# kris927b/TextBlaster

Measured on AMD Instinct MI355X. Metric: documents/sec through full C4+Gopher+langID pipeline at 1/2/4/8 MI355X, higher is better.
Workload: dtype bf16

## Files before the change

csrc/common/devplan.h:

```cpp
#pragma once
#include "tb_common.h"

namespace tb {

constexpr int kMaxStageSteps = 8;
constexpr int kMaxNgramEntries = 16;
constexpr int kMaxStopChars = 16;
constexpr int kMaxStopWords = 512;
constexpr int kStopTableSize = 2048;
constexpr int kStopBlobBytes = 16384;

enum DevStepKind : int32_t {
  DK_NONE = 0,
  DK_GOPHER_QUALITY = 1,
  DK_GOPHER_REP = 2,
  DK_FINEWEB = 3,
  DK_LANGID = 4,
};

constexpr uint32_t kC4MaxGrowth = 16;

struct DevStep {
  int32_t kind;
  int32_t width;
  int64_t rec_base;
  int32_t rec_prefix;
  int32_t stop_set;
  int32_t n_top, n_dup;
  int32_t top_n[kMaxNgramEntries];
  int32_t dup_n[kMaxNgramEntries];
  int32_t n_stop_chars;
  uint32_t stop_chars[kMaxStopChars];
  int64_t short_line_length;
};

constexpr int kStopLiteMaxSlots = 256;
constexpr int kStopLiteMaxWords = 64;
constexpr int kStopLiteMaxBlob = 1024;

TB_HD uint32_t stop_lite_hash_push(uint32_t h, uint8_t v) { return (h ^ v) * 16777619u; }
constexpr uint32_t kStopLiteHash0 = 2166136261u;
TB_HD uint32_t stop_lite_slot(uint32_t h, uint32_t nslots) { return (h * 0x9E3779B1u) & (nslots - 1); }

struct DevStopSet {
  uint64_t keys[kStopTableSize];
  int32_t idx[kStopTableSize];
  int32_t off[kMaxStopWords + 1];
  int32_t n;
  int32_t max_len;
  uint8_t blob[kStopBlobBytes];
  int32_t lite_nslots;
  uint32_t lite_slots[kStopLiteMaxSlots];
  uint64_t fast_keys[kStopLiteMaxSlots];
  int32_t all_ascii7;
};

TB_HD uint32_t stop_fast_slot(uint64_t key, uint32_t nslots) {
  uint64_t h = key * 0x9E3779B97F4A7C15ull;
  return (uint32_t)(h >> 40) & (nslots - 1);
}

struct DevC4 {
  int32_t split_paragraph, remove_citations, filter_no_terminal_punct;
  int32_t filter_lorem_ipsum, filter_javascript, filter_curly_bracket, filter_policy;
  int64_t min_words_per_line, max_word_length;
  int64_t min_num_sentences;
};

struct DevStage {
  int32_t n_steps;
  int32_t width_total;
  DevStep steps[kMaxStageSteps];
};

constexpr int kMaxStopSets = 4;

struct DevPlan {
  int32_t n_stop_sets;
  DevStopSet stops[kMaxStopSets];
};

constexpr uint64_t kScratchPerByte = 80;
constexpr uint64_t kScratchPerByteSplit = 176;
TB_HD uint64_t scratch_bytes_for_dev(uint32_t doc_len, bool split = false) {
  return (split ? kScratchPerByteSplit : kScratchPerByte) * ((uint64_t)doc_len + 64) + 4096;
}

TB_HD uint64_t dev_key(uint64_t h, uint32_t len) {
  uint64_t x = h ^ ((uint64_t)len * 0xD6E8FEB86659FD93ull);
  x ^= x >> 33;
  x *= 0xff51afd7ed558ccdull;
  x ^= x >> 33;
  x *= 0xc4ceb9fe1a85ec53ull;
  x ^= x >> 33;
  return x | 1ull;
}

constexpr uint32_t kNoWords = 0xFFFFFFFFu;
struct DictLines {
  const int64_t* off = nullptr;
  const uint32_t* data = nullptr;
  TB_HD const uint32_t* at(uint32_t d) const { return (off && off[d] >= 0) ? data + off[d] : nullptr; }
};
struct DictIn {
  const int64_t* moff = nullptr;
  const uint32_t* bits = nullptr;
  const uint32_t* words = nullptr;
  TB_HD const uint32_t* marks(uint32_t d) const { return (moff && moff[d] >= 0) ? bits + moff[d] : nullptr; }
  TB_HD uint32_t nwords(uint32_t d) const { return words ? words[d] : kNoWords; }
};

}
```

csrc/common/docproc.h:

```cpp
#pragma once
#include <type_traits>

#include "devplan.h"
#include "hash.h"
#include "langid.h"
#include "par.h"
#include "uax29.h"
#include "ucd.h"

namespace tb {

enum : int {
  PH_START = 0, PH_DECODE, PH_DICT, PH_PREFIX_HASH, PH_WORDS, PH_LINES, PH_GQ, PH_GR_LINES, PH_GR_WORDS,
  PH_GR_TOP, PH_GR_DUP, PH_FW, PH_LID, PH_GR_DUP_WALK, PH_GR_DUP_CANON, PH_GR_TOP_CANON,
  PH_C4_LOREM = 16, PH_C4_DECODE, PH_C4_LINES, PH_C4_CITE, PH_C4_WORDS, PH_C4_CODES, PH_C4_JOIN, PH_C4_SENT,
  PH_GR_NL = 24, PH_GR_LINE_DUP, PH_GR_WH, PH_GR_WCANON, PH_GQ_WORDS, PH_GQ_BYTES, PH_RUST_LINES,
  kPhaseSlots = 32
};

enum : uint32_t {
  DOC_OK = 0,
  DOC_NEEDS_CPU = 1,
  DOC_OVERFLOW = 2,
};

constexpr uint32_t P16_CASE_IGN = 1u << 14;
TB_HD uint16_t compact_prop(uint32_t p) {
  return (uint16_t)((p & 0xBFFFu) | ((p & P_CASE_IGN) ? P16_CASE_IGN : 0u));
}

struct PropArr {
  const uint32_t* ent = nullptr;
  const uint16_t* p16 = nullptr;
  TB_HD uint32_t operator[](uint32_t i) const { return ent ? (ent[i] >> 16) : (uint32_t)p16[i]; }
  TB_HD PropArr operator+(uint32_t s) const { return PropArr{ent ? ent + s : nullptr, ent ? nullptr : p16 + s}; }
};
struct OffArr {
  const uint32_t* ent = nullptr;
  const uint32_t* o32 = nullptr;
  TB_HD uint32_t operator[](uint32_t i) const { return ent ? (ent[i] & 0xFFFFu) : o32[i]; }
};

struct Cps {
  uint32_t n = 0;
  uint32_t* ent = nullptr;
  uint32_t* off = nullptr;
  uint16_t* prop = nullptr;
  const uint8_t* b = nullptr;
  uint32_t nb = 0;
  TB_HD PropArr props() const { return PropArr{ent, prop}; }
  TB_HD OffArr offs() const { return OffArr{ent, off}; }
  TB_HD uint32_t o(uint32_t i) const { return ent ? (ent[i] & 0xFFFFu) : off[i]; }
  TB_HD uint32_t p(uint32_t i) const { return ent ? (ent[i] >> 16) : (uint32_t)prop[i]; }
  TB_HD uint8_t lead(uint32_t i) const { return b[o(i)]; }
  TB_HD bool is_lf(uint32_t i) const { return (p(i) & P_WB_MASK) == (uint32_t)WB_LF; }
  TB_HD uint32_t cp(uint32_t i) const {
    int len;
    return utf8_decode(b, o(i), nb, &len);
  }
};

struct CpsAcc {
  PropArr prop;
  TB_HD uint32_t p(int i) const { return prop[(uint32_t)i]; }
};

struct PHView {
  const uint64_t* ph8 = nullptr;
  uint64_t phn = 0;
  const uint8_t* b = nullptr;
  uint32_t n = 0;
  TB_HD uint64_t at(uint32_t x) const {
    if (x >= n) return phn;
    uint64_t h = ph8[x >> 3];
    for (uint32_t j = x & ~7u; j < x; ++j) h = hash_push(h, b[j]);
    return h;
  }
};

struct PreDoc {
  uint32_t* off;
  uint16_t* prop;
  uint32_t* wbm;
  uint32_t* nl_pos;
  uint32_t* nl_len;
  uint32_t n;
  uint32_t C;
  uint32_t dict;
  uint32_t NL;
  uint32_t tcs;
  uint32_t tce;
  uint32_t nl_a;
  uint32_t nl_e;
  uint32_t* wtmp;
  uint32_t* wcs;
  uint32_t* wce;
  uint32_t* wbs;
  uint32_t* wbe;
  uint8_t* wal;
  uint32_t W;
  uint32_t pad;
  uint64_t* wh;
  uint64_t* wtab;
  uint64_t* wk;
  uint64_t* wpb;
  uint64_t* wcsum;
  uint32_t* wslot;
  uint32_t* wid;
  uint32_t* wl;
  uint32_t wready;
  uint32_t pad2;
};

struct Words {
  uint32_t n = 0;
  uint32_t* cs = nullptr;
  uint32_t* ce = nullptr;
  uint32_t* bs = nullptr;
  uint32_t* be = nullptr;
  uint8_t* alpha = nullptr;
};

struct Lines {
  uint32_t n = 0;
  uint32_t* ls = nullptr;
  uint32_t* le = nullptr;
};

struct HL {
  uint64_t h;
  uint32_t len;
  uint32_t pad;
};

template <class P>
struct DocCtx {
  P par;
  UcdView ucd;
  const uint64_t* pw = nullptr;
  const uint64_t* ipw = nullptr;
  uint32_t pw_n = 0;
// ... 68 lines not shown
    uint64_t a = (used + 15) & ~15ull;
    uint64_t e = a + count * sizeof(T) + 16;
    if (e > cap) {
      overflow = true;
      return (T*)scr;
    }
    used = a + count * sizeof(T);
    if constexpr (P::kWaves == 0) {
      if (used > peak) peak = used;
    }
    return (T*)(scr + a);
  }
  TB_HD void set_flag(uint32_t f) {
    if (flag) P::or32(flag, f);
  }
  TB_HD uint64_t powb(uint32_t k) const { return k <= pw_n ? pw[k] : hpow(kHashBase, k); }
  TB_HD uint64_t ipowb(uint32_t k) const { return (ipw && k <= pw_n) ? ipw[k] : hpow(kHashBaseInv, k); }
  template <class T>
  TB_HD T* try_lds(uint64_t count) {
    if (!lds) return nullptr;
    const uint64_t a = (lused + 15u) & ~15u;
    const uint64_t e = a + count * sizeof(T);
    if (e + lhi > lcap) return nullptr;
    lused = (uint32_t)e;
    return (T*)(lds + a);
  }
};

TB_HD bool is_ws(uint32_t p) { return (p & P_WS) != 0; }

template <class P, class PA>
TB_HD void trim_span(DocCtx<P>& x, const PA& prop, uint32_t C, uint32_t& tcs, uint32_t& tce) {
#if defined(__HIPCC__)
  if constexpr (P::kWaves == 1) {
    const uint32_t lane = x.par.lane;
    tcs = C;
    for (uint32_t base = 0; base < C; base += 64) {
      const uint32_t j = base + lane;
      const uint64_t m = __ballot(j < C && !is_ws(prop[j]));
      if (m) { tcs = base + (uint32_t)__builtin_ctzll(m); break; }
    }
    tce = 0;
    if (tcs < C) {
      for (uint32_t base = (C - 1) & ~63u;; base -= 64) {
        const uint32_t j = base + lane;
        const uint64_t m = __ballot(j < C && !is_ws(prop[j]));
        if (m) { tce = base + (uint32_t)(64 - __clzll((long long)m)); break; }
        if (base == 0) break;
      }
    }
    return;
  }
#endif
  tcs = x.par.template min<uint32_t>(C, C, [&](uint32_t i) { return is_ws(prop[i]) ? C : i; });
  tce = x.par.template max<uint32_t>(C, 0u, [&](uint32_t i) { return is_ws(prop[i]) ? 0u : i + 1; });
}
constexpr uint32_t kWave16 = 43000;
TB_HD constexpr int rec_gr_fixed() { return 7; }

template <class P>
TB_HD Cps decode(DocCtx<P>& x, const uint8_t* b, uint32_t n, bool hot = false, uint32_t* dict = nullptr) {
  Cps c;
  c.b = b;
  c.nb = n;
  const bool packed = n < 65536u;
  if (packed) {
    c.ent = hot ? x.template alloc_hot_hi<uint32_t>(n + 1) : x.template alloc<uint32_t>(n + 1);
  } else {
    c.prop = hot ? x.template alloc_hot_hi<uint16_t>(n + 1) : x.template alloc<uint16_t>(n + 1);
    c.off = hot ? x.template alloc_hot_hi<uint32_t>(n + 1) : x.template alloc<uint32_t>(n + 1);
  }
  if (x.overflow) return c;
  const UcdView ucd = x.ucd;
  const uint16_t* asc = x.asc;
  uint32_t* ent = c.ent;
  uint32_t* off = c.off;
  uint16_t* pra = c.prop;
  uint32_t dl = 0;
  c.n = x.par.template compact<int>(
      n, [&](uint32_t i, int&) { return utf8_is_lead(b[i]); },
      [&](uint32_t i, uint32_t k, int&) {
        uint16_t cpk;
        const uint32_t c0 = b[i];
        if (asc && (c0 < 0x80 || (c0 & 0xFEu) == 0xC2u)) {
          cpk = asc[c0 < 0x80 ? c0 : (((c0 & 0x1Fu) << 6) | (b[i + 1] & 0x3Fu))];
        } else {
          int len;
          const uint32_t p = ucd.props(utf8_decode(b, i, n, &len));
          cpk = compact_prop(p);
          dl |= (p & P_DICT) ? 1u : 0u;
        }
        if (packed) {
          ent[k] = i | ((uint32_t)cpk << 16);
        } else {
          off[k] = i;
          pra[k] = cpk;
        }
      });
  const uint32_t cn = c.n;
  x.par.single([&]() {
    if (packed) ent[cn] = n;
    else { off[cn] = n; pra[cn] = 0; }
  });
  if (dict) *dict = x.par.reduce_or(dl);
  x.par.sync();
  return c;
}

template <class P>
TB_HD uint64_t span_hash8(const DocCtx<P>& x, const PHView& v, uint32_t s, uint32_t e) {
  const uint64_t hs = v.at(s), he = v.at(e);
  return he - hs * x.powb(e - s);
}

template <class P>
TB_HD PHView prefix_hash8(DocCtx<P>& x, const uint8_t* b, uint32_t n) {
  PHView v;
  v.b = b;
  v.n = n;
  const uint32_t nblk = (n + 7) >> 3;
  uint64_t* ph8 = x.template alloc_hot_hi<uint64_t>(nblk + 1);
  if (x.overflow) return v;
  const uint64_t* pw = x.pw;
  const uint32_t pwn = x.pw_n;
  HL tot = x.par.template scan<HL>(
      nblk, HL{0, 0, 0},
      [&](const HL& a, const HL& c) {
        uint64_t m = c.len <= pwn ? pw[c.len] : hpow(kHashBase, c.len);
        return HL{a.h * m + c.h, a.len + c.len, 0};
      },
      [&](uint32_t k) {
        const uint32_t s0 = k << 3, e0 = s0 + 8 < n ? s0 + 8 : n;
        uint64_t h = 0;
        for (uint32_t j = s0; j < e0; ++j) h = hash_push(h, b[j]);
        return HL{h, e0 - s0, 0};
      },
      [&](uint32_t k, const HL& e) { ph8[k] = e.h; });
  x.par.single([&]() { ph8[nblk] = tot.h; });
  x.par.sync();
  v.ph8 = ph8;
  v.phn = tot.h;
  return v;
}

struct WSeg {
  uint32_t bits;
  uint32_t first;
  uint32_t last;
};
TB_HD WSeg wseg_op(const WSeg& a, const WSeg& b) {
  if (b.bits & 1u) return b;
  return WSeg{a.bits | (b.bits & 6u), a.first < b.first ? a.first : b.first, a.last > b.last ? a.last : b.last};
}

#ifndef TB_WB_CTX
#define TB_WB_CTX 1
#endif
#if defined(__HIPCC__)
static __constant__ WbPairTab g_wb_pair_tab = kWbPairTab;
#endif
TB_HD bool word_mark(const PropArr& prop, uint32_t C, uint32_t i) {
  if (i == 0 || i == C) return true;
  if (TB_WB_CTX) {
    const uint32_t pm2 = i >= 2 ? prop[i - 2] : 0xFFFFFFFFu;
    const uint32_t pp1 = i + 1 < C ? prop[i + 1] : 0xFFFFFFFFu;
#if defined(__HIP_DEVICE_COMPILE__)
    const int r = wb_break_ctx_tab(pm2, prop[i - 1], prop[i], pp1, [](uint32_t k) { return g_wb_pair_tab.w[k]; });
// ... 362 lines not shown
    while (true) {
      uint64_t cur = tab[slot];
      if (cur == 0) {
        cur = P::cas64(&tab[slot], 0, mine);
        if (cur == 0) break;
      }
      if ((cur >> 32) == fp) {
        if ((cur & 0xFFFFFFFFull) > (uint64_t)i + 1u) P::min64(&tab[slot], mine);
        break;
      }
      if (++slot == capn) slot = 0;
    }
    canon[i] = slot;
  });
  x.par.sync();
  bool collided = false;
  x.par.for_n(n, [&](uint32_t i) {
    uint32_t c = (uint32_t)(tab[canon[i]] & 0xFFFFFFFFull) - 1u;
    if (c != i && !eq(i, c)) { collided = true; c = i; }
    canon[i] = c;
    res(i, c);
  });
  if (collided) x.set_flag(DOC_NEEDS_CPU);
  x.par.sync();
  x.reset(mark);
}

template <class P, class KeyF, class EqF, class CT>
TB_HD void canonicalize(DocCtx<P>& x, uint32_t n, KeyF&& key, EqF&& eq, CT* canon) {
  canonicalize_res(x, n, key, eq, canon, NoResolve{});
}

template <class P>
TB_HD bool bytes_eq(const uint8_t* b, uint32_t a0, uint32_t a1, uint32_t b0, uint32_t b1) {
  if (a1 - a0 != b1 - b0) return false;
  const uint32_t n = a1 - a0;
  uint32_t i = 0;
  for (; i + 16 <= n; i += 16) {
    uint32_t diff = 0;
#pragma unroll
    for (uint32_t k = 0; k < 16; ++k) diff |= (uint32_t)(b[a0 + i + k] ^ b[b0 + i + k]);
    if (diff) return false;
  }
  uint32_t diff = 0;
  for (; i < n; ++i) diff |= (uint32_t)(b[a0 + i] ^ b[b0 + i]);
  return diff == 0;
}

template <class P, class SpanF>
TB_HD void dup_spans(DocCtx<P>& x, const uint8_t* b, const PHView& ph, uint32_t n, SpanF&& span,
                     int64_t* out_elems, int64_t* out_bytes) {
  if (n <= 1) {
    *out_elems = 0;
    *out_bytes = 0;
    return;
  }
  const auto mark = x.mark();
  uint32_t* canon = x.template alloc_hot<uint32_t>(n + 1);
  if (x.overflow) return;
  canonicalize(
      x, n,
      [&](uint32_t i) {
        uint32_t s, e;
        span(i, s, e);
        return dev_key(span_hash8(x, ph, s, e), e - s);
      },
      [&](uint32_t i, uint32_t j) {
        uint32_t s0, e0, s1, e1;
        span(i, s0, e0);
        span(j, s1, e1);
        return bytes_eq<P>(b, s0, e0, s1, e1);
      },
      canon);
  *out_elems = x.par.template sum<int64_t>(n, [&](uint32_t i) { return canon[i] != i ? (int64_t)1 : (int64_t)0; });
  *out_bytes = x.par.template sum<int64_t>(n, [&](uint32_t i) {
    if (canon[i] == i) return (int64_t)0;
    uint32_t s, e;
    span(i, s, e);
    return (int64_t)(e - s);
  });
  x.reset(mark);
}

template <class F>
TB_HD void lower_bytes(const UcdView& ucd, const Cps& cv, uint32_t s, uint32_t e, F&& push) {
  uint8_t buf[4];
  const PropArr prop = cv.props();
  for (uint32_t k = s; k < e; ++k) {
    uint32_t c = cv.cp(k);
    uint32_t lc;
    if (c == 0x3A3) {
      bool before = false, after = false;
      for (uint32_t j = k; j > s; --j) {
        uint32_t p = prop[j - 1];
        if (p & P16_CASE_IGN) continue;
        before = (p & P_CASED) != 0;
        break;
      }
      for (uint32_t j = k + 1; j < e; ++j) {
        uint32_t p = prop[j];
        if (p & P16_CASE_IGN) continue;
        after = (p & P_CASED) != 0;
        break;
      }
      lc = (before && !after) ? 0x3C2 : 0x3C3;
    } else {
      lc = ucd.lower(c);
    }
    int nb = utf8_encode(lc, buf);
    for (int q = 0; q < nb; ++q) push(buf[q]);
    if (c == 0x130) { push(0xCC); push(0x87); }
  }
}

TB_HD bool is_stop_word(const UcdView& ucd, const DevStopSet& ss, const Cps& cv, uint32_t s, uint32_t e,
                        uint32_t b0, uint32_t b1) {
  if (ss.n == 0 || (int32_t)(e - s) > ss.max_len) return false;
  if (ss.lite_nslots > 0) {
    const uint32_t nb = b1 - b0;
    if (nb <= 7u && nb == e - s) {
      uint64_t key = (uint64_t)nb << 56;
      for (uint32_t k = 0; k < nb; ++k) {
        uint32_t c = cv.b[b0 + k];
        if (c >= 'A' && c <= 'Z') c += 32;
        key |= (uint64_t)c << (8 * k);
      }
      const uint32_t ns = (uint32_t)ss.lite_nslots;
      uint32_t slot = stop_fast_slot(key, ns);
      while (true) {
        const uint64_t f = ss.fast_keys[slot];
        if (f == 0) return false;
        if (f == key) return true;
        slot = (slot + 1) & (ns - 1);
      }
    }
    if (ss.all_ascii7) {
      bool e2 = false;
      for (uint32_t k = b0; k < b1; ++k) e2 |= cv.b[k] == 0xE2;
      if (!e2) return false;
    }
  }
  uint64_t h = 0;
  uint32_t len = 0;
  lower_bytes(ucd, cv, s, e, [&](uint8_t v) { h = hash_push(h, v); ++len; });
  const uint64_t key = dev_key(h, len);
  uint32_t slot = (uint32_t)(key >> 17) & (kStopTableSize - 1);
  while (true) {
    const uint64_t k = ss.keys[slot];
    if (k == 0) return false;
    if (k == key) {
      const int32_t w = ss.idx[slot];
      const int32_t o0 = ss.off[w], o1 = ss.off[w + 1];
      if ((uint32_t)(o1 - o0) != len) return false;
      int32_t pos = o0;
      bool ok = true;
      lower_bytes(ucd, cv, s, e, [&](uint8_t v) { ok = ok && ss.blob[pos++] == v; });
      return ok;
    }
    slot = (slot + 1) & (kStopTableSize - 1);
  }
}

TB_HD bool ci_contains(const uint8_t* b, uint32_t n, const char* pat, int plen) {
  for (uint32_t s = 0; s < n; ++s) {
    uint32_t i = s;
    int j = 0;
    for (; j < plen; ++j) {
      if (i >= n) break;
      const char pc = pat[j];
      uint8_t c = b[i];
      if (c >= 'A' && c <= 'Z') c = (uint8_t)(c + 32);
      if (c == (uint8_t)pc) { ++i; continue; }
      if (pc == 'k' && i + 2 < n && b[i] == 0xE2 && b[i + 1] == 0x84 && b[i + 2] == 0xAA) { i += 3; continue; }
      break;
    }
    if (j == plen) return true;
  }
  return false;
}

struct GrExport {
  const uint32_t* wid;
  const uint32_t* WL;
  const uint64_t* K;
  const uint64_t* PB;
  const uint32_t* bs;
  const uint32_t* be;
  const uint8_t* b;
  char* free_base;
  uint64_t free_cap;
  uint32_t W;
  uint32_t valid;
  const uint32_t* rs;
  const uint32_t* rl;
  const uint32_t* prs;
  OffArr off;
  PHView ph;
  uint32_t NR, NPR, tcs, tce;
  uint32_t lines_valid;
};

TB_HD void gr_line_span(const uint32_t* rs, const uint32_t* rl, const OffArr& off, uint32_t tcs, uint32_t tce,
                        uint32_t NR, uint32_t k, uint32_t& s0, uint32_t& e0) {
  const uint32_t cs = k == 0 ? tcs : rs[k - 1] + rl[k - 1];
  const uint32_t ce = k == NR ? tce : rs[k];
  s0 = off[cs];
  e0 = off[ce];
}
TB_HD void gr_para_span(const uint32_t* rs, const uint32_t* rl, const uint32_t* prs, const OffArr& off,
                        uint32_t tcs, uint32_t tce, uint32_t NPR, uint32_t q, uint32_t& s0, uint32_t& e0) {
  const uint32_t cs = q == 0 ? tcs : rs[prs[q - 1]] + rl[prs[q - 1]];
  const uint32_t ce = q == NPR ? tce : rs[prs[q]];
  s0 = off[cs];
  e0 = off[ce];
}

struct StageOut {
  int64_t* rec;
  uint32_t ndocs;
  uint32_t doc;
  GrExport* gr_export = nullptr;
  uint32_t* line_stats = nullptr;
  const PreDoc* pre = nullptr;
  const uint8_t* b_global = nullptr;
  DictIn dict;
};

constexpr uint32_t kLineStatsNone = 0xFFFFFFFFu;
struct alignas(16) LineStat { uint32_t bs, be, nw, mx; };
TB_HD uint64_t line_stats_base(int64_t off_d, int64_t d) { return 4ull * ((uint64_t)off_d / 8u + 16ull * (uint64_t)d); }
TB_HD uint32_t line_stats_cap(uint32_t n) { return n / 8u + 15u; }
TB_HD uint64_t line_stats_words(const int64_t* off, int64_t ndocs) {
  return line_stats_base(off[ndocs], ndocs) + 16u;
}

template <class P>
TB_HD void export_line_stats(DocCtx<P>& x, const Cps& c, const Words& w, const Lines& L, uint32_t n, uint32_t* out) {
  const uint32_t NL = L.n;
  if (NL > line_stats_cap(n) || x.overflow) return;
  const auto mark = x.mark();
  uint32_t* ls = x.template alloc_hot<uint32_t>(NL + 1);
  uint32_t* nw = x.template alloc_hot<uint32_t>(NL + 1);
  uint32_t* mx = x.template alloc_hot<uint32_t>(NL + 1);
  if (x.overflow) {
    x.overflow = false;
    x.reset(mark);
    return;
  }
  const PropArr prop = c.props();
  const OffArr off = c.offs();
  x.par.for_n(NL, [&](uint32_t k) { ls[k] = L.ls[k]; nw[k] = 0; mx[k] = 0; });
  x.par.sync();
  x.par.for_n(w.n, [&](uint32_t q) {
    const uint32_t cs = w.cs[q];
    uint32_t lo = 0, hi = NL;
    while (hi - lo > 1) {
      const uint32_t mid = (lo + hi) >> 1;
      if (ls[mid] <= cs) lo = mid; else hi = mid;
    }
    P::add32(&nw[lo], 1u);
    P::max32(&mx[lo], w.ce[q] - cs);
  });
  x.par.sync();
  LineStat* st = (LineStat*)(out + 4);
  x.par.for_n(NL, [&](uint32_t k) {
    uint32_t s0 = ls[k], e0 = L.le[k];
    while (s0 < e0 && is_ws(prop[s0])) ++s0;
    while (e0 > s0 && is_ws(prop[e0 - 1])) --e0;
    st[k] = LineStat{off[s0], off[e0], nw[k], mx[k]};
  });
  x.par.sync();
  x.par.single([&]() { out[0] = NL; });
  x.reset(mark);
}

struct DupGrams {
  const uint32_t* wid;
  const uint32_t* WL;
  const uint64_t* K;
  const uint64_t* PB;
  const uint32_t* bs;
  const uint32_t* be;
// ... 80 lines not shown
      g = gc[p];
      len = WL[p + n] - WL[p];
    }
    const bool seen0 =
        act && ((__hip_atomic_load(&sn[g >> 5], __ATOMIC_RELAXED, __HIP_MEMORY_SCOPE_AGENT) >> (g & 31)) & 1u);
    uint64_t A = __ballot(act), S = __ballot(seen0), cnt = 0, fv = 0;
    uint32_t next = p0 + 64;
    while (A) {
      const uint32_t k = (uint32_t)__builtin_ctzll(A);
      if ((S >> k) & 1ull) {
        cnt |= 1ull << k;
        const uint32_t j = k + n;
        A = j >= 64 ? 0ull : (A & (~0ull << j));
        if (p0 + j > next) next = p0 + j;
      } else {
        fv |= 1ull << k;
        S |= __ballot(g == (uint32_t)__builtin_amdgcn_readlane((int)g, (int)k));
        A &= A - 1;
      }
    }
    if ((fv >> lane) & 1ull) atomicOr(&sn[g >> 5], 1u << (g & 31));
    uint32_t add = ((cnt >> lane) & 1ull) ? len : 0u;
    for (int o = 32; o > 0; o >>= 1) add += (uint32_t)__shfl_xor((int)add, o);
    rep += add;
    __builtin_amdgcn_fence(__ATOMIC_RELEASE, "workgroup");
    __builtin_amdgcn_fence(__ATOMIC_ACQUIRE, "workgroup");
    idx = next;
  }
  return rep;
#else
  (void)par;
  return dup_walk(G, n, gc, R, sn, WL);
#endif
}

TB_HD uint64_t span_hash(uint64_t pa, uint64_t pb, uint64_t blen_pow) {
  return pb - pa * blen_pow;
}

template <class P>
TB_HD uint32_t count_sentences_upto(DocCtx<P>& x, const Cps& c, uint32_t s, uint32_t e, uint32_t limit) {
  const uint32_t m = e - s;
  if (m == 0 || limit == 0) return 0;
  constexpr uint32_t kChunk = 256;
  const auto mark = x.mark();
  uint32_t* starts = x.template alloc_hot<uint32_t>(kChunk + 1);
  uint32_t* segf = x.template alloc_hot<uint32_t>(kChunk + 1);
  if (x.overflow) return 0;
  const PropArr prop = c.props() + s;
  CpsAcc acc{prop};
  uint32_t cnt = 0;
  bool seen = false;
  for (uint32_t base = 0; base < m && cnt < limit; base += kChunk) {
    const uint32_t len = m - base < kChunk ? m - base : kChunk;
    const uint32_t NS = x.par.template compact<int>(
        len, [&](uint32_t i, int&) { const uint32_t g = base + i; return g == 0 || sb_break(acc, (int)m, (int)g); },
        [&](uint32_t i, uint32_t k, int&) { starts[k] = i; });
    x.par.sync();
    const uint32_t first = NS ? starts[0] : len;
    const bool lead_any = x.par.template sum<uint32_t>(first, [&](uint32_t i) {
      return is_ws(prop[base + i]) ? 0u : 1u;
    }) != 0;
    const uint32_t segs = x.par.template sum<uint32_t>(NS, [&](uint32_t k) {
      const uint32_t a = starts[k], bnd = k + 1 < NS ? starts[k + 1] : len;
      uint32_t f = 0;
      for (uint32_t j = a; j < bnd; ++j) if (!is_ws(prop[base + j])) { f = 1; break; }
      segf[k] = f;
      return f;
    });
    x.par.sync();
    if (!seen && lead_any) ++cnt;
    cnt += segs;
    seen = NS ? segf[NS - 1] != 0 : (seen || lead_any);
    x.par.sync();
  }
  x.reset(mark);
  return cnt;
}

template <class P>
TB_HD void gopher_rep_record(DocCtx<P>& x, const DevStep& ds, const uint8_t* b, const Cps& c,
                             const PHView& ph, const Words& w, int64_t* r, bool release_props = false,
                             GrExport* ex = nullptr, const PreDoc* pre = nullptr,
                             const uint8_t* b_export = nullptr, Lines lines = Lines{}) {
  const uint32_t C = c.n;
  const PropArr prop = c.props();
  const OffArr off = c.offs();
  const int width = ds.width;
  uint32_t tcs, tce;
  trim_span(x, prop, C, tcs, tce);
  if (tcs >= tce) {
    x.par.single([&]() {
      for (int k = 0; k < width; ++k) r[k] = 0;
      r[0] = -1;
    });
    return;
  }
  const auto mark = x.mark();
  const uint32_t span = tce - tcs;
  uint32_t* rs;
  uint32_t* rl;
  uint32_t NR;
  if (pre) {
    const uint32_t a = pre->nl_a, e = pre->nl_e;
    rs = pre->nl_pos + a;
    rl = pre->nl_len + a;
    NR = e - a;
  } else if (lines.n > 0) {
    const uint32_t* ls = lines.ls;
    const uint32_t NL = lines.n;
    rs = P::kWaves == 1 ? x.template alloc_hot<uint32_t>(NL + 1) : x.template alloc<uint32_t>(NL + 1);
    rl = P::kWaves == 1 ? x.template alloc_hot<uint32_t>(NL + 1) : x.template alloc<uint32_t>(NL + 1);
    if (x.overflow) return;
    NR = x.par.template compact<int>(
        NL,
        [&](uint32_t k, int&) {
          if (k == 0) return false;
          const uint32_t p = ls[k] - 1;
          return p >= tcs && p < tce && (k == 1 || ls[k - 1] != p);
        },
        [&](uint32_t k, uint32_t q, int&) {
          uint32_t e = k;
          while (e + 1 < NL && ls[e + 1] == ls[e] + 1) ++e;
          rs[q] = ls[k] - 1;
          rl[q] = e - k + 1;
        });
    x.par.sync();
  } else {
    rs = x.template alloc<uint32_t>(span + 1);
    rl = x.template alloc<uint32_t>(span + 1);
    if (x.overflow) return;
    NR = x.par.template compact<int>(
        span,
        [&](uint32_t i, int&) {
          const uint32_t j = tcs + i;
          return c.is_lf(j) && !c.is_lf(j - 1);
        },
        [&](uint32_t i, uint32_t k, int&) {
          uint32_t j = tcs + i, q = j;
          while (c.is_lf(q)) ++q;
          rs[k] = j;
          rl[k] = q - j;
        });
    x.par.sync();
  }
  x.stamp(PH_GR_NL);
  uint32_t* prs = x.template alloc<uint32_t>(NR + 1);
  if (x.overflow) return;
  int64_t line_dup = 0, line_dup_b = 0, para_dup = 0, para_dup_b = 0;
#ifdef TB_NO_SPLIT_LINES
  const bool split_lines = false;
#else
  const bool split_lines = ex && P::kWaves != 1 && !x.in_lds(rs) && !x.in_lds(rl) && !x.in_lds(prs) &&
                           !x.in_lds(ph.ph8) && !x.in_lds(c.ent) && !x.in_lds(c.off);
#endif
  if (!split_lines)
    dup_spans(x, b, ph, NR + 1,
              [&](uint32_t k, uint32_t& s0, uint32_t& e0) { gr_line_span(rs, rl, off, tcs, tce, NR, k, s0, e0); },
              &line_dup, &line_dup_b);
  x.stamp(PH_GR_LINE_DUP);
  const uint32_t NPR = x.par.template compact<int>(
      NR, [&](uint32_t k, int&) { return rl[k] >= 2; }, [&](uint32_t k, uint32_t q, int&) { prs[q] = k; });
  x.par.sync();
  if (!split_lines)
    dup_spans(x, b, ph, NPR + 1,
              [&](uint32_t q, uint32_t& s0, uint32_t& e0) {
                gr_para_span(rs, rl, prs, off, tcs, tce, NPR, q, s0, e0);
              },
              &para_dup, &para_dup_b);
  if (ex) {
    x.par.single([&]() {
// ... 414 lines not shown
        part[D - 1] += lid_grams_n(lid_letter(ucd, b, n, p3), lid_letter(ucd, b, n, p2),
                                   lid_letter(ucd, b, n, p1), l0, [&](uint32_t g, int order) {
                                     lid_add_emb(lt.E, g, order, part);
                                   });
      },
      tmp, sums);
  x.reset(mark);
}

template <class P>
TB_HD void langid_record(DocCtx<P>& x, const uint8_t* b, uint32_t n, const LidTables& lt, int64_t* r) {
  const auto mark = x.mark();
  int64_t* sums = x.template alloc_hot<int64_t>(kLidDim + 1);
  if (x.overflow) return;
  langid_sums<P, kLidDim + 1>(x, b, n, lt, sums);
  if (x.overflow) return;
  x.par.single([&]() { lid_record_v3(sums, sums[kLidDim], lt, r); });
  x.par.sync();
  x.reset(mark);
}

TB_HD bool end_punct(uint32_t c) {
  return c == '.' || c == '!' || c == '?' || c == '"' || c == '\'' || c == 0x201D;
}

TB_HD bool ci_starts_with(const uint8_t* b, uint32_t n, const char* pat, int plen) {
  uint32_t i = 0;
  for (int j = 0; j < plen; ++j) {
    if (i >= n) return false;
    const char pc = pat[j];
    uint8_t c = b[i];
    if (c >= 'A' && c <= 'Z') c = (uint8_t)(c + 32);
    if (c == (uint8_t)pc) { ++i; continue; }
    if (pc == 'k' && i + 2 < n && b[i] == 0xE2 && b[i + 1] == 0x84 && b[i + 2] == 0xAA) { i += 3; continue; }
    return false;
  }
  return true;
}

TB_HD uint32_t lower3(const uint8_t* b, uint32_t n) {
  uint32_t w = 0;
#pragma unroll
  for (uint32_t k = 0; k < 3; ++k) {
    uint32_t c = k < n ? b[k] : 0u;
    if (c >= 'A' && c <= 'Z') c += 32;
    w |= c << (8 * k);
  }
  return w;
}
TB_HD constexpr uint32_t pack3(const char* p) {
  return (uint32_t)(uint8_t)p[0] | ((uint32_t)(uint8_t)p[1] << 8) | ((uint32_t)(uint8_t)p[2] << 16);
}

enum : uint32_t { C4F_JS = 1, C4F_POLICY = 2 };

enum : uint32_t { C4S_LOREM = 4, C4S_CURLY = 8, C4S_CITE = 16 };

TB_HD uint32_t c4_phrases_at(const DevC4& c4, const uint8_t* b, uint32_t n, uint32_t s) {
  uint8_t c0 = b[s];
  if (c0 >= 'A' && c0 <= 'Z') c0 = (uint8_t)(c0 + 32);
  if (c0 != 'j' && c0 != 't' && c0 != 'p' && c0 != 'c' && c0 != 'u') return 0;
  const char* const kPol[6] = {"terms of use", "privacy policy", "cookie policy",
                               "uses cookies", "use of cookies", "use cookies"};
  const int kPolLen[6] = {12, 14, 13, 12, 14, 11};
  uint32_t bits = 0;
  const uint32_t w3 = lower3(b + s, n - s);
  auto pre = [&](const char* pat) { return w3 == pack3(pat); };
  if (c4.filter_javascript && c0 == 'j' && pre("javascript") && ci_starts_with(b + s, n - s, "javascript", 10))
    bits |= C4F_JS;
  if (c4.filter_policy)
    for (int t = 0; t < 6; ++t)
      if (kPol[t][0] == (char)c0 && pre(kPol[t]) && ci_starts_with(b + s, n - s, kPol[t], kPolLen[t])) {
        bits |= C4F_POLICY;
        break;
      }
  return bits;
}

TB_HD uint32_t swar_eq_mask(uint32_t v, uint32_t c) {
  const uint32_t t = v ^ (c * 0x01010101u);
  return ~(((t & 0x7F7F7F7Fu) + 0x7F7F7F7Fu) | t | 0x7F7F7F7Fu);
}

template <class P>
TB_HD uint64_t gq_byte_counts(DocCtx<P>& x, const uint8_t* b, uint32_t n) {
  const uintptr_t a0 = (uintptr_t)b & ~(uintptr_t)3;
  const uint32_t head = (uint32_t)((uintptr_t)b - a0);
  const uint32_t nd = (head + n + 3) >> 2;
  const uint32_t* w = (const uint32_t*)a0;
  auto dw = [&](int64_t k) -> uint32_t {
    if (k < 0 || k >= (int64_t)nd) return 0u;
    const int64_t e = 4 * k + 4 - head;
    if (e <= (int64_t)n && 4 * k >= (int64_t)head) return w[k];
    uint32_t v = 0;
    for (uint32_t j = 0; j < 4; ++j) {
      const int64_t sj = 4 * k + j - head;
      if (sj >= 0 && sj < (int64_t)n) v |= (uint32_t)b[sj] << (8 * j);
    }
    return v;
  };
  return x.par.template sum<uint64_t>((nd + 3) >> 2, [&](uint32_t g) {
    uint32_t d[6];
#pragma unroll
    for (uint32_t i = 0; i < 6; ++i) d[i] = dw((int64_t)4 * g + i - 1);
    uint64_t acc = 0;
#pragma unroll
    for (uint32_t i = 0; i < 4; ++i) {
      const uint32_t v = d[i + 1];
      acc += (uint64_t)__builtin_popcount(swar_eq_mask(v, '#')) << 32;
      const uint32_t dots = swar_eq_mask(v, '.'), e2 = swar_eq_mask(v, 0xE2);
      if ((dots | e2) == 0) continue;
      const uint64_t v64 = (uint64_t)v | ((uint64_t)d[i + 2] << 32);
      for (uint32_t r = 0; r < 4; ++r) {
        const uint32_t c0 = (v >> (8 * r)) & 0xFFu;
        if (c0 == 0xE2) {
          acc += ((v64 >> (8 * r + 8)) & 0xFFFFu) == 0xA680u ? 1u : 0u;
          continue;
        }
        if (c0 != '.') continue;
        const uint32_t prev = r ? (v >> (8 * r - 8)) & 0xFFu : d[i] >> 24;
        if (prev == '.') continue;
        uint32_t len = 1;
        while (r + len < 8 && ((v64 >> (8 * (r + len))) & 0xFFu) == '.') ++len;
        if (r + len == 8) {
          int64_t j = 4 * ((int64_t)4 * g + i) + r + len - head;
          while (j < (int64_t)n && b[j] == '.') { ++j; ++len; }
        }
        acc += len / 3;
      }
    }
    return acc;
  });
}

TB_HD uint64_t swar_lower8(uint64_t v) {
  constexpr uint64_t k7F = 0x7F7F7F7F7F7F7F7Full, k80 = 0x8080808080808080ull;
  const uint64_t ge_a = (v & k7F) + 0x3F3F3F3F3F3F3F3Full;
  const uint64_t gt_z = (v & k7F) + 0x2525252525252525ull;
  const uint64_t upper = ge_a & ~gt_z & ~v & k80;
  return v | (upper >> 2);
}

template <class P, class F>
TB_HD void scan_bytes16(DocCtx<P>& x, const uint8_t* b, uint32_t n, F&& f) {
  const uintptr_t a0 = (uintptr_t)b & ~(uintptr_t)3;
  const uint32_t head = (uint32_t)((uintptr_t)b - a0);
  const uint32_t nd = (head + n + 3) >> 2;
  const uint32_t* w = (const uint32_t*)a0;
  auto dw = [&](uint32_t k) -> uint32_t {
    if (k >= nd) return 0u;
    const int64_t e = (int64_t)4 * k + 4 - head;
    if (e <= (int64_t)n && 4 * k >= head) return w[k];
    uint32_t v = 0;
    for (uint32_t j = 0; j < 4; ++j) {
      const int64_t sj = (int64_t)4 * k + j - head;
      if (sj >= 0 && sj < (int64_t)n) v |= (uint32_t)b[sj] << (8 * j);
    }
    return v;
  };
  x.par.for_n((nd + 3) >> 2, [&](uint32_t g) {
    uint32_t d[5];
#pragma unroll
    for (uint32_t i = 0; i < 5; ++i) d[i] = dw(4 * g + i);
#pragma unroll
    for (uint32_t i = 0; i < 4; ++i) {
      const uint32_t k = 4 * g + i;
      const uint64_t v = (uint64_t)d[i] | ((uint64_t)d[i + 1] << 32);
      const uint64_t lo = swar_lower8(v);
      for (uint32_t r = 0; r < 4; ++r) {
        const int64_t sp = (int64_t)4 * k + r - head;
        if (sp < 0 || sp >= (int64_t)n) continue;
        f((uint32_t)sp, (uint32_t)(v >> (8 * r)) & 0xFFu, (uint32_t)(v >> (8 * r + 8)) & 0xFFu,
          (uint32_t)(lo >> (8 * r)) & 0xFFFFFFu);
      }
    }
  });
}

TB_HD bool c4_phrase_prefix(uint32_t l3) {
  return l3 == pack3("jav") || l3 == pack3("ter") || l3 == pack3("pri") || l3 == pack3("coo") || l3 == pack3("use");
}

template <class P>
TB_HD uint32_t c4_byte_scan(DocCtx<P>& x, const DevC4& c4, const uint8_t* b, uint32_t n) {
  uint32_t acc = 0;
  const bool phrases = c4.filter_javascript || c4.filter_policy;
  scan_bytes16(x, b, n, [&](uint32_t s, uint32_t c0, uint32_t c1, uint32_t l3) {
    if (c4.filter_curly_bracket && (c0 == '{' || c0 == '}')) acc |= C4S_CURLY;
    if (c0 == '[' && ((c1 >= '0' && c1 <= '9') || c1 >= 0x80)) acc |= C4S_CITE;
    if (c4.filter_lorem_ipsum && l3 == pack3("lor") && ci_starts_with(b + s, n - s, "lorem ipsum", 11))
      acc |= C4S_LOREM;
    if (phrases && c4_phrase_prefix(l3)) acc |= c4_phrases_at(c4, b, n, s);
  });
  return x.par.reduce_or(acc);
}

template <class P>
TB_HD void c4_finish(DocCtx<P>& x, const DevC4& c4, uint32_t n, uint8_t* Jb, uint32_t Jtot, int64_t s_long,
                     int64_t s_punct, int64_t s_few, int64_t* r, int64_t* src) {
  Cps jc = decode(x, Jb, Jtot);
  if (x.overflow) { x.set_flag(DOC_NEEDS_CPU | DOC_OVERFLOW); return; }
  const uint32_t JC = jc.n;
  const PropArr jprop = jc.props();
  uint32_t tcs, tce;
  trim_span(x, jprop, JC, tcs, tce);
  uint32_t nsent = 0, bstart = 0, blen = 0;
  if (tcs < tce) {
    const uint32_t lim = c4.min_num_sentences > 0xFFFFFFFFll ? 0xFFFFFFFFu : (uint32_t)c4.min_num_sentences;
    nsent = count_sentences_upto(x, jc, tcs, tce, lim);
    bstart = jc.o(tcs);
    blen = jc.o(tce) - jc.o(tcs);
  }
  x.stamp(PH_C4_SENT);
  const int64_t jrel = (int64_t)((const char*)Jb - x.scr) + bstart;
// ... 580 lines not shown
      x.par.sync();
      x.reset(mc);
    }
  } else {
    Cps pc = decode(x, Pb, Ptot);
    Words pwd = words(x, pc);
    if (!line_arrays() || x.overflow) { x.set_flag(DOC_NEEDS_CPU | DOC_OVERFLOW); return; }
    x.par.for_n(pwd.n, [&](uint32_t q) {
      const uint32_t lo = line_of_byte(pwd.bs[q]);
      P::add32(&nw[lo], 1u);
      P::max32(&mx[lo], pwd.ce[q] - pwd.cs[q]);
    });
  }
  x.stamp(PH_C4_WORDS);
  if (c4.filter_javascript || c4.filter_policy) {
    scan_bytes16(x, Pb, Ptot, [&](uint32_t s, uint32_t, uint32_t, uint32_t l3) {
      if (!c4_phrase_prefix(l3)) return;
      const uint32_t bits = c4_phrases_at(c4, Pb, Ptot, s);
      if (bits) P::or32(&pf[line_of_byte(s)], bits);
    });
  }
  x.par.sync();
  x.par.for_n(NLn, [&](uint32_t k) {
    const uint8_t* lp = Pb + poff[k];
    const uint32_t ln = plen[k];
    uint8_t cd = 0;
    if (c4.max_word_length > 0 && (int64_t)mx[k] > c4.max_word_length) {
      cd = 1;
    } else if (c4.filter_no_terminal_punct) {
      bool term = false;
      if (ln > 0) {
        uint32_t st = ln - 1;
        while (st > 0 && (lp[st] & 0xC0) == 0x80) --st;
        int len;
        term = end_punct(utf8_decode(lp, st, ln, &len));
      }
      const bool ell = ln >= 3 && lp[ln - 1] == '.' && lp[ln - 2] == '.' && lp[ln - 3] == '.';
      if (!term || ell) cd = 2;
    }
    if (cd == 0 && c4.min_words_per_line > 0 && (int64_t)nw[k] < c4.min_words_per_line) cd = 3;
    if (cd == 0 && c4.filter_javascript && (pf[k] & C4F_JS)) cd = 4;
    if (cd == 0 && c4.filter_policy && (pf[k] & C4F_POLICY)) cd = 5;
    code[k] = cd;
  });
  x.par.sync();
  const int64_t s_long = x.par.template sum<int64_t>(NLn, [&](uint32_t k) { return (int64_t)(code[k] == 1); });
  const int64_t s_punct = x.par.template sum<int64_t>(NLn, [&](uint32_t k) { return (int64_t)(code[k] == 2); });
  const int64_t s_few = x.par.template sum<int64_t>(NLn, [&](uint32_t k) { return (int64_t)(code[k] == 3); });
  if (wout && hls) {
    const uint32_t wk = x.par.template sum<uint32_t>(NLn, [&](uint32_t k) { return code[k] == 0 ? nw[k] : 0u; });
    x.par.single([&]() { *wout = wk; });
  }
  x.stamp(PH_C4_CODES);
  uint32_t* joff = x.template alloc_hot<uint32_t>(NLn + 1);
  if (x.overflow) { x.set_flag(DOC_NEEDS_CPU | DOC_OVERFLOW); return; }
  uint32_t Jtot = x.par.template scan<uint32_t>(
      NLn, 0u, [](uint32_t a, uint32_t b2) { return a + b2; },
      [&](uint32_t k) { return code[k] == 0 ? plen[k] + 1 : 0u; }, [&](uint32_t k, uint32_t e) { joff[k] = e; });
  if (Jtot > 0) Jtot -= 1;
  uint8_t* Jb = x.template alloc_global<uint8_t>(Jtot + 1);
  if (x.overflow) { x.set_flag(DOC_NEEDS_CPU | DOC_OVERFLOW); return; }
  x.par.sync();
  x.par.for_n(C, [&](uint32_t j) {
    const uint32_t nb = kept_bytes(j);
    if (!nb || code[lid[j]] != 0) return;
    const uint32_t k = lid[j];
    uint8_t* d = Jb + joff[k] + (Pw[j] - Pw[la[k]]);
    for (uint32_t q = 0; q < nb; ++q) d[q] = b[off[j] + q];
  });
  x.par.for_n(NLn, [&](uint32_t k) {
    if (code[k] == 0 && joff[k] + plen[k] < Jtot) Jb[joff[k] + plen[k]] = '\n';
  });
  x.par.sync();
  x.stamp(PH_C4_JOIN);
  c4_finish(x, c4, n, Jb, Jtot, s_long, s_punct, s_few, r, src);
}


#ifndef TB_HOT_PROPS
#define TB_HOT_PROPS 1
#endif
constexpr bool kHotProps = TB_HOT_PROPS != 0;

template <class P, bool kWithLid = true, bool kPre = false>
TB_HD void analyze_stage(DocCtx<P>& x, const DevStage& st, const DevPlan& plan,
                         const LidTables& lid, const uint8_t* b, uint32_t n, StageOut& out) {
  bool need_words = false, need_lines = false, need_ph = false, need_lid = false;
  for (int s = 0; s < st.n_steps; ++s) {
    const int k = st.steps[s].kind;
    if (k == DK_GOPHER_QUALITY) need_words = need_lines = true;
    if (k == DK_GOPHER_REP) need_words = need_ph = true;
    if (k == DK_FINEWEB) need_words = need_lines = need_ph = true;
    if (k == DK_LANGID) need_lid = true;
  }
  x.stamp(PH_START);
  if (out.line_stats) x.par.single([&]() { out.line_stats[0] = kLineStatsNone; });
  uint32_t ndict = 0;
  Cps c;
  if constexpr (kPre) {
    c.n = out.pre->C;
    c.off = out.pre->off;
    c.prop = out.pre->prop;
    c.b = b;
    c.nb = n;
    ndict = out.pre->dict;
  } else {
    c = decode(x, b, n, kHotProps, &ndict);
  }
  if (x.overflow) { x.set_flag(DOC_NEEDS_CPU | DOC_OVERFLOW); return; }
  x.stamp(PH_DECODE);
  const uint32_t C = c.n;
  const uint32_t* dict_marks = nullptr;
  uint32_t wfix = kNoWords;
  if (ndict && need_words) {
    bool fw_only = true;
    for (int s = 0; s < st.n_steps; ++s)
      fw_only &= st.steps[s].kind != DK_GOPHER_QUALITY && st.steps[s].kind != DK_GOPHER_REP;
    if (!kPre) dict_marks = out.dict.marks(out.doc);
    if (!kPre && !dict_marks && fw_only) wfix = out.dict.nwords(out.doc);
    if (!dict_marks && wfix == kNoWords) {
      if constexpr (kWithLid) {
        for (int s = 0; s < st.n_steps; ++s) {
          const DevStep& ds = st.steps[s];
          if (ds.kind == DK_LANGID && lid.E)
            langid_record(x, b, n, lid, out.rec + (int64_t)ds.rec_prefix * out.ndocs + (int64_t)out.doc * ds.width);
        }
      }
      x.set_flag(DOC_NEEDS_CPU);
      return;
    }
  }
  x.stamp(PH_DICT);
  PHView ph;
  if (need_ph) ph = prefix_hash8(x, b, n);
  x.stamp(PH_PREFIX_HASH);
  Words w;
  if (need_words) {
    w = words(x, c, kPre ? out.pre : nullptr, dict_marks);
  }
  x.stamp(PH_WORDS);
  Lines L;
  if (need_lines) L = rust_lines(x, c);
  if (x.overflow) { x.set_flag(DOC_NEEDS_CPU | DOC_OVERFLOW); return; }
  x.stamp(PH_RUST_LINES);
  if (out.line_stats && need_words && need_lines) export_line_stats(x, c, w, L, n, out.line_stats);
  x.stamp(PH_LINES);
  const uint32_t W = w.n;
  const PropArr prop = c.props();
  const OffArr off = c.offs();

  int n_gr = 0;
  for (int s = 0; s < st.n_steps; ++s) n_gr += st.steps[s].kind == DK_GOPHER_REP;
  int gr_seen = 0;
  for (int so = 0; so < 2 * st.n_steps; ++so) {
    const int s = so % st.n_steps;
    const DevStep& ds = st.steps[s];
    if ((so < st.n_steps) == (ds.kind == DK_GOPHER_REP)) continue;
    int64_t* r = out.rec + (int64_t)ds.rec_prefix * out.ndocs + (int64_t)out.doc * ds.width;
    if (ds.kind == DK_GOPHER_QUALITY) {
      const DevStopSet& ss = plan.stops[ds.stop_set];
      const UcdView ucd = x.ucd;
      auto lo32 = [](uint64_t v) { return (int64_t)(v & 0xFFFFFFFFull); };
      auto hi32 = [](uint64_t v) { return (int64_t)(v >> 32); };
      int64_t sum_chars = 0;
      const uint64_t as = x.par.template sum<uint64_t>(W, [&](uint32_t k) {
        const uint32_t a = w.cs[k], e = w.ce[k];
        return ((uint64_t)(e - a) << 32) | ((uint64_t)w.alpha[k] << 16) |
               (uint64_t)is_stop_word(ucd, ss, c, a, e, w.bs[k], w.be[k]);
      });
      int64_t alpha, stop;
      if (W < 65536u) {
        sum_chars = hi32(as);
        alpha = (int64_t)((as >> 16) & 0xFFFFull);
        stop = (int64_t)(as & 0xFFFFull);
      } else {
        sum_chars = x.par.template sum<int64_t>(W, [&](uint32_t k) { return (int64_t)(w.ce[k] - w.cs[k]); });
        alpha = x.par.template sum<int64_t>(W, [&](uint32_t k) { return (int64_t)w.alpha[k]; });
        stop = x.par.template sum<int64_t>(W, [&](uint32_t k) {
          return (int64_t)is_stop_word(ucd, ss, c, w.cs[k], w.ce[k], w.bs[k], w.be[k]);
        });
      }
      x.stamp(PH_GQ_WORDS);
      const uint64_t he = P::kWaves <= 1 ? gq_byte_counts(x, b, n) : x.par.template sum<uint64_t>(n, [&](uint32_t i) {
        const uint32_t c0 = b[i];
        if (c0 == '#') return (uint64_t)1 << 32;
        if (c0 == 0xE2) return (uint64_t)(i + 2 < n && b[i + 1] == 0x80 && b[i + 2] == 0xA6);
        if (c0 != '.' || (i > 0 && b[i - 1] == '.')) return (uint64_t)0;
        uint32_t j = i;
        while (j < n && b[j] == '.') ++j;
        return (uint64_t)((j - i) / 3);
      });
      x.stamp(PH_GQ_BYTES);
      const int64_t nhash = hi32(he), nell = lo32(he);
      const uint64_t be = x.par.template sum<uint64_t>(L.n, [&](uint32_t k) {
        const uint32_t ls = L.ls[k], le = L.le[k];
        uint32_t j = ls;
        while (j < le && is_ws(prop[j])) ++j;
        const uint32_t l0 = j < le ? c.lead(j) : 0u;
        const uint64_t bul = (l0 == '-' || (l0 == 0xE2 && c.cp(j) == 0x2022)) ? 1 : 0;
        j = le;
        while (j > ls && is_ws(prop[j - 1])) --j;
        const uint32_t E = off[j], S = off[ls];
        uint64_t ell = 0;
        if (E - S >= 3) {
          const bool dots = b[E - 3] == '.' && b[E - 2] == '.' && b[E - 1] == '.';
          const bool uell = b[E - 3] == 0xE2 && b[E - 2] == 0x80 && b[E - 1] == 0xA6;
          ell = (dots || uell) ? 1 : 0;
        }
        return (bul << 32) | ell;
      });
      const int64_t bullet = hi32(be), ell_lines = lo32(be);
      x.par.single([&]() {
        r[0] = W; r[1] = sum_chars; r[2] = nhash; r[3] = nell; r[4] = L.n;
        r[5] = bullet; r[6] = ell_lines; r[7] = alpha; r[8] = stop;
      });
      x.stamp(PH_GQ);
    } else if (ds.kind == DK_GOPHER_REP) {
      ++gr_seen;
      gopher_rep_record(x, ds, b, c, ph, w, r, kHotProps && gr_seen == n_gr, n_gr == 1 ? out.gr_export : nullptr,
                        kPre ? out.pre : nullptr, out.b_global, L);
    } else if (ds.kind == DK_FINEWEB) {
      const auto mark = x.mark();
      uint32_t* nb = x.template alloc<uint32_t>(L.n + 1);
      if (x.overflow) { x.set_flag(DOC_NEEDS_CPU | DOC_OVERFLOW); return; }
      const uint32_t NB = x.par.template compact<int>(
          L.n,
          [&](uint32_t k, int&) {
            for (uint32_t j = L.ls[k]; j < L.le[k]; ++j) if (!is_ws(prop[j])) return true;
            return false;
          },
          [&](uint32_t k, uint32_t q, int&) { nb[q] = k; });
      x.par.sync();
      int64_t stop_end = x.par.template sum<int64_t>(NB, [&](uint32_t q) {
        uint32_t k = nb[q];
        uint32_t j = L.le[k];
        while (j > L.ls[k] && is_ws(prop[j - 1])) --j;
        uint32_t last = c.cp(j - 1);
        for (int t = 0; t < ds.n_stop_chars; ++t) if (ds.stop_chars[t] == last) return (int64_t)1;
        return (int64_t)0;
      });
      int64_t shrt = x.par.template sum<int64_t>(NB, [&](uint32_t q) {
        uint32_t k = nb[q];
        return (int64_t)((int64_t)(L.le[k] - L.ls[k]) <= ds.short_line_length);
      });
      int64_t dup_e = 0, dup_b = 0;
      dup_spans(x, b, ph, NB,
                [&](uint32_t q, uint32_t& s0, uint32_t& e0) { s0 = off[L.ls[nb[q]]]; e0 = off[L.le[nb[q]]]; },
                &dup_e, &dup_b);
      int64_t nl = x.par.template sum<int64_t>(C, [&](uint32_t i) { return (int64_t)c.is_lf(i); });
      x.par.single([&]() {
        r[0] = NB; r[1] = stop_end; r[2] = shrt; r[3] = dup_b; r[4] = (int64_t)C - nl; r[5] = nl; r[6] = W;
      });
      x.reset(mark);
      x.stamp(PH_FW);
    } else if (ds.kind == DK_LANGID) {
      if constexpr (kWithLid)
        if (lid.E) langid_record(x, b, n, lid, r);
      x.stamp(PH_LID);
    }
    if (x.overflow) { x.set_flag(DOC_NEEDS_CPU | DOC_OVERFLOW); return; }
  }
  if (wfix != kNoWords) {
    x.par.sync();
    x.par.single([&]() {
      for (int s = 0; s < st.n_steps; ++s) {
        const DevStep& ds = st.steps[s];
        if (ds.kind == DK_FINEWEB) out.rec[(int64_t)ds.rec_prefix * out.ndocs + (int64_t)out.doc * ds.width + 6] = wfix;
      }
      if (out.line_stats) out.line_stats[0] = kLineStatsNone;
    });
  }
}

}
```

csrc/hip/kernels.hip:

```cpp
#include <hip/hip_runtime.h>
#include <algorithm>
#include <cstdlib>
#include <string>

#include "../common/docproc.h"
#include "../common/gate.h"
#include "../common/badwords.h"

using namespace tb;

namespace {

constexpr uint32_t kMaxLdsPerDoc = 160 * 1024;
constexpr uint32_t kMaxLdsPerBlk = 128 * 1024;

struct DevTables {
  const uint16_t* s1;
  const uint32_t* s2;
  const uint16_t* l1;
  const int32_t* l2;
};

extern __shared__ __attribute__((aligned(16))) char g_lds_arena[];

template <class P = WavePar>
__device__ __forceinline__ DocCtx<P> make_ctx(const DevTables& t, const uint64_t* pw, uint32_t pw_n,
                                             char* scratch, const int64_t* scratch_off, int doc, int k,
                                             uint32_t* flags, uint32_t lds_bytes, uint64_t* prof) {
  DocCtx<P> x;
  x.prof = prof ? prof + (size_t)doc * kPhaseSlots : nullptr;
  x.lds = lds_bytes ? (char*)g_lds_arena : nullptr;
  x.lcap = lds_bytes;
  x.lused = 0;
  x.ucd = UcdView{t.s1, t.s2, t.l1, t.l2};
  x.pw = pw;
  x.pw_n = pw_n;
  x.ipw = pw ? pw + pw_n + 1 : nullptr;
  x.scr = scratch + scratch_off[k];
  x.cap = (uint64_t)(scratch_off[k + 1] - scratch_off[k]);
  x.used = 0;
  x.flag = flags + doc;
  return x;
}

template <class P>
__device__ __forceinline__ void lds_ascii_props(DocCtx<P>& x) {
  uint16_t* asc = x.template try_lds<uint16_t>(256);
  if (!asc) return;
  x.par.for_n(256, [&](uint32_t c) { asc[c] = compact_prop(x.ucd.props(c)); });
  x.par.sync();
  x.asc = asc;
}

template <class P>
__device__ __forceinline__ const uint8_t* lds_text(DocCtx<P>& x, const uint8_t* b, uint32_t n) {
  const uintptr_t a0 = (uintptr_t)b & ~(uintptr_t)3;
  const uint32_t head = (uint32_t)((uintptr_t)b - a0);
  const uint32_t nd = (head + n + 3) >> 2;
  uint32_t* d = x.template try_lds<uint32_t>(nd + 1);
  if (!d) return b;
  const uint32_t* src = (const uint32_t*)a0;
  x.par.for_n(nd, [&](uint32_t k) { d[k] = src[k]; });
  x.par.sync();
  return (const uint8_t*)d + head;
}

template <class P>
__device__ __forceinline__ void c4_src_absolute(DocCtx<P>& x, int64_t* src, int64_t slice_begin) {
  if (x.par.leader() && src[0] >= 0) src[0] += slice_begin;
}

#define TB_STAGE_KERNEL(NAME, ATTR)                                                                   \
  __global__ __launch_bounds__(64) ATTR void NAME(                                                   \
      const DevPlan* __restrict__ plan, const DevStage* __restrict__ stage, const uint8_t* __restrict__ bytes, \
      const int64_t* __restrict__ off, const int32_t* __restrict__ perm, int32_t ndocs, char* scratch,        \
      const int64_t* __restrict__ scratch_off, const uint64_t* __restrict__ pw, uint32_t pw_n, DevTables tabs, \
      int64_t* rec, uint32_t* flags, uint32_t lds_bytes, uint64_t* prof,                               \
      const uint8_t* __restrict__ dead, uint32_t* line_stats, GrExport* gr_export, DictIn dict) {      \
    const int doc = perm ? perm[blockIdx.x] : (int)blockIdx.x;                                        \
    if (doc >= ndocs || (dead && dead[doc])) return;                                                  \
    DocCtx<WavePar> x = make_ctx(tabs, pw, pw_n, scratch, scratch_off, doc, (int)blockIdx.x, flags, lds_bytes, prof);   \
    const uint32_t n = (uint32_t)(off[doc + 1] - off[doc]);                                           \
    lds_ascii_props(x);                                                                               \
    const uint8_t* b = lds_text(x, bytes + off[doc], n);                                              \
    StageOut out{rec, (uint32_t)ndocs, (uint32_t)doc};                                                \
    if (line_stats) out.line_stats = line_stats + line_stats_base(off[doc], doc);                     \
    if (gr_export) { out.gr_export = gr_export + blockIdx.x; out.b_global = bytes + off[doc]; }       \
    out.dict = dict;                                                                                  \
    analyze_stage<WavePar, false>(x, *stage, *plan, LidTables{}, b, n, out);  \
  }

#ifndef TB_STAGE_WPE
#define TB_STAGE_WPE 8
#endif
TB_STAGE_KERNEL(k_stage_analyze_wave, __attribute__((amdgpu_waves_per_eu(TB_STAGE_WPE, 8))))

#ifndef TB_BLOCK_THREADS
#define TB_BLOCK_THREADS 512
#endif
constexpr int kBlockThreads = TB_BLOCK_THREADS;
#ifndef TB_BLK_WPE
#define TB_BLK_WPE 6
#endif
#if TB_BLK_WPE > 0
#define TB_BLK_ATTR __attribute__((amdgpu_waves_per_eu(TB_BLK_WPE, 8)))
#else
#define TB_BLK_ATTR
#endif
__shared__ __attribute__((aligned(16))) char g_block_xs[16 * (kBlockThreads / 64) + 64];

template <int NT, bool kPre = false>
__device__ __forceinline__ void stage_blk_body(
    const DevPlan* __restrict__ plan, const DevStage* __restrict__ stage, const uint8_t* __restrict__ bytes,
    const int64_t* __restrict__ off, const int32_t* __restrict__ perm, int32_t ndocs, char* scratch,
    const int64_t* __restrict__ scratch_off, const uint64_t* __restrict__ pw, uint32_t pw_n, DevTables tabs,
    int64_t* rec, uint32_t* flags, uint32_t lds_bytes, uint64_t* prof, const uint8_t* __restrict__ dead,
    GrExport* gr_export, int32_t n_split, uint32_t split_bytes, uint32_t* line_stats, const PreDoc* pre,
    int32_t n_pre, DictIn dict) {
  const int doc = perm[blockIdx.x];
  if (doc >= ndocs || (dead && dead[doc])) return;
  DocCtx<BlockPar<NT>> x =
      make_ctx<BlockPar<NT>>(tabs, pw, pw_n, scratch, scratch_off, doc, (int)blockIdx.x, flags, lds_bytes, prof);
  x.par.xs = g_block_xs;
  lds_ascii_props(x);
  const uint8_t* b = bytes + off[doc];
  const uint32_t n = (uint32_t)(off[doc + 1] - off[doc]);
  StageOut out{rec, (uint32_t)ndocs, (uint32_t)doc};
  out.dict = dict;
  if (line_stats) out.line_stats = line_stats + line_stats_base(off[doc], doc);
  if constexpr (kPre) {
    if (pre[blockIdx.x].n != n) return;
    out.pre = pre + blockIdx.x;
  }
  if (gr_export && (int)blockIdx.x < n_split && n > split_bytes) out.gr_export = gr_export + blockIdx.x;
  analyze_stage<BlockPar<NT>, false, kPre>(x, *stage, *plan, LidTables{}, b, n, out);
}

#define TB_STAGE_BLK_KERNEL(NAME, NT, PRE)                                                             \
  __global__ __launch_bounds__(NT) TB_BLK_ATTR void NAME(                                            \
      const DevPlan* __restrict__ plan, const DevStage* __restrict__ stage, const uint8_t* __restrict__ bytes, \
      const int64_t* __restrict__ off, const int32_t* __restrict__ perm, int32_t ndocs, char* scratch,         \
      const int64_t* __restrict__ scratch_off, const uint64_t* __restrict__ pw, uint32_t pw_n, DevTables tabs,  \
      int64_t* rec, uint32_t* flags, uint32_t lds_bytes, uint64_t* prof, const uint8_t* __restrict__ dead,   \
      GrExport* gr_export, int32_t n_split, uint32_t split_bytes, uint32_t* line_stats,                \
      const PreDoc* pre, int32_t n_pre, DictIn dict) {                                                 \
    stage_blk_body<NT, PRE>(plan, stage, bytes, off, perm, ndocs, scratch, scratch_off, pw, pw_n, tabs, rec, flags, \
                       lds_bytes, prof, dead, gr_export, n_split, split_bytes, line_stats, pre, n_pre, dict); \
  }
TB_STAGE_BLK_KERNEL(k_stage_analyze_blk, kBlockThreads, false)
TB_STAGE_BLK_KERNEL(k_stage_analyze_blk_pre, kBlockThreads, true)

__global__ __launch_bounds__(kBlockThreads) TB_BLK_ATTR void k_gr_dup_split(
    const DevStage* __restrict__ stage, int32_t gr_step, const int32_t* __restrict__ perm, int32_t n_split,
    int32_t n_tasks, int32_t ndocs, const GrExport* __restrict__ ex, const uint64_t* __restrict__ pw, uint32_t pw_n,
    DevTables tabs, int64_t* rec, uint32_t* flags, uint32_t lds_bytes, uint32_t* cursor) {
  __shared__ int s_task;
  const int total = n_split * n_tasks;
  const DevStep& ds = stage->steps[gr_step];
  while (true) {
    if (threadIdx.x == 0) s_task = (int)atomicAdd(cursor, 1u);
    __syncthreads();
    const int task = s_task;
    __syncthreads();
    if (task >= total) break;
    const int k = task / n_tasks, t = task % n_tasks;
    const int doc = perm[k];
    if (doc >= ndocs) continue;
    const GrExport e = ex[k];
    if (!e.valid) continue;
    DocCtx<BlockPar<kBlockThreads>> x;
    x.prof = nullptr;
    x.lds = lds_bytes ? (char*)g_lds_arena : nullptr;
    x.lcap = lds_bytes;
    x.lused = 0;
    x.ucd = UcdView{tabs.s1, tabs.s2, tabs.l1, tabs.l2};
    x.pw = pw;
    x.pw_n = pw_n;
    x.ipw = pw ? pw + pw_n + 1 : nullptr;
// ... 1233 lines not shown
      d.wpb[k] = pow_at(pw, pw_n, wl);
      uint32_t cc = (uint32_t)(d.wtab[d.wslot[k]] & 0xFFFFFFFFull) - 1u;
      if (cc != k && !bytes_eq<WavePar>(b, d.wbs[k], d.wbe[k], d.wbs[cc], d.wbe[cc])) {
        bad = true;
        cc = k;
      }
      d.wid[k] = cc;
      wl += len[j];
      tsum += d.wh[k] * ipow_at(pw, pw_n, wl);
    }
    if (bad) atomicOr(&flags[doc], DOC_NEEDS_CPU);
    uint64_t ttot;
    (void)pre_block_scan<uint64_t>(tsum, sh, &ttot);
    if (threadIdx.x == 0) {
      if (nch) d.wcsum[2 * nch + c] = ttot;
      if (c + 1 >= nch) {
        const uint32_t total = (uint32_t)((nch ? d.wcsum[nch + c] : 0ull) + tot);
        d.wl[W] = total;
        d.wpb[W] = pow_at(pw, pw_n, total);
      }
    }
    return;
  }
  uint32_t wl = (uint32_t)lbase;
  uint64_t t[kPreWPer];
  uint64_t tsum = 0;
#pragma unroll
  for (uint32_t j = 0; j < kPreWPer; ++j) {
    const uint32_t k = t0 + j;
    wl += len[j];
    t[j] = k < W ? d.wh[k] * ipow_at(pw, pw_n, wl) : 0ull;
    tsum += t[j];
  }
  uint64_t ttot;
  uint64_t kb = (nch ? d.wcsum[3 * nch + c] : 0ull) + pre_block_scan<uint64_t>(tsum, sh, &ttot);
#pragma unroll
  for (uint32_t j = 0; j < kPreWPer; ++j) {
    const uint32_t k = t0 + j;
    if (k >= W) break;
    d.wk[k] = kb;
    kb += t[j];
  }
  if (threadIdx.x == 0 && c + 1 >= nch) d.wk[W] = (nch ? d.wcsum[3 * nch + c] : 0ull) + ttot;
}

template <int MODE>
__global__ __launch_bounds__(64) void k_pre_wsum(const int32_t* __restrict__ perm, const uint8_t* __restrict__ dead,
                                                 PreDoc* pre) {
  const uint32_t s = blockIdx.x;
  if (dead && dead[perm[s]]) return;
  const PreDoc d = pre[s];
  const uint32_t nch = (d.W + kPreWChunk - 1) / kPreWChunk;
  const uint32_t lane = threadIdx.x;
  const uint64_t* in = d.wcsum + (MODE ? 2 * nch : 0);
  uint64_t* out = d.wcsum + (MODE ? 3 * nch : nch);
  uint64_t carry = 0;
  for (uint32_t b0 = 0; b0 < nch; b0 += 64) {
    const uint32_t q = b0 + lane;
    const uint64_t v = q < nch ? in[q] : 0ull;
    const uint64_t incl = pardetail::wave_incl_scan(v, lane, [](uint64_t a, uint64_t b) { return a + b; });
    if (q < nch) out[q] = carry + incl - v;
    carry += pardetail::bcast63(incl);
  }
  if (MODE == 1 && lane == 0) pre[s].wready = 1;
}

}

static int device_cus() {
  static const int cus = [] {
    int dev = 0, n = 0;
    if (hipGetDevice(&dev) != hipSuccess || hipDeviceGetAttribute(&n, hipDeviceAttributeMultiprocessorCount, dev) !=
        hipSuccess || n <= 0)
      n = 256;
    return n;
  }();
  return cus;
}

extern "C" {

int tb_scan_strided_i64(hipStream_t stream, const int64_t* src, int64_t stride, int64_t n, int64_t* out);

int tb_stage_analyze(hipStream_t stream, const void* plan, const void* stage, const uint8_t* bytes,
                     const int64_t* off, const int32_t* perm, int32_t ndocs, char* scratch,
                     const int64_t* scratch_off, const uint64_t* pw, uint32_t pw_n, const uint16_t* s1,
                     const uint32_t* s2, const uint16_t* l1, const int32_t* l2, int64_t* rec, uint32_t* flags,
                     uint32_t lds_bytes, uint64_t* prof, int32_t waves, int32_t nblocks, const uint8_t* dead,
                     uint32_t* line_stats, void* gr_export, const int64_t* dict_moff, const uint32_t* dict_bits,
                     const uint32_t* dict_words) {
  if (ndocs <= 0) return 0;
  if (nblocks <= 0) nblocks = ndocs;
  if (lds_bytes > kMaxLdsPerDoc) return (int)hipErrorInvalidValue;
  DevTables t{s1, s2, l1, l2};
  if (waves != TB_STAGE_WPE) return (int)hipErrorInvalidValue;
  auto kern = k_stage_analyze_wave;
  if (lds_bytes > 65536)
    (void)hipFuncSetAttribute((const void*)kern, hipFuncAttributeMaxDynamicSharedMemorySize, (int)lds_bytes);
  hipLaunchKernelGGL(kern, dim3(nblocks), dim3(64), lds_bytes, stream, (const DevPlan*)plan,
                     (const DevStage*)stage, bytes, off, perm, ndocs, scratch, scratch_off, pw, pw_n, t, rec, flags,
                     lds_bytes, prof, dead, line_stats, (GrExport*)gr_export, DictIn{dict_moff, dict_bits, dict_words});
  return (int)hipGetLastError();
}

int tb_gr_split_wave(hipStream_t stream, const void* stage, int32_t gr_step, const int32_t* perm, int32_t n_docs,
                     int32_t n_tasks, int32_t ndocs, const void* gr_export, const uint64_t* pw, uint32_t pw_n,
                     const uint16_t* s1, const uint32_t* s2, const uint16_t* l1, const int32_t* l2, int64_t* rec,
                     uint32_t* flags, uint32_t lds_bytes, int32_t block, uint64_t* prof, int32_t n_big) {
  if (n_docs <= 0 || n_tasks <= 0) return 0;
  if (!perm || !gr_export || gr_step < 0 || gr_step >= kMaxStageSteps || n_tasks > 2 * kMaxNgramEntries ||
      lds_bytes > kMaxLdsPerDoc || n_big < 0 || n_big > n_docs)
    return (int)hipErrorInvalidValue;
  DevTables t{s1, s2, l1, l2};
  const GrExport* ex = (const GrExport*)gr_export;
  const int32_t n_wave = block ? n_big : n_docs;
  if (n_wave > 0) {
    if (lds_bytes > 65536)
      (void)hipFuncSetAttribute((const void*)k_gr_split_wave, hipFuncAttributeMaxDynamicSharedMemorySize,
                                (int)lds_bytes);
    hipLaunchKernelGGL(k_gr_split_wave, dim3((uint32_t)n_wave * (uint32_t)n_tasks), dim3(64), lds_bytes, stream,
                       (const DevStage*)stage, gr_step, perm, n_tasks, ndocs, ex, pw, pw_n, t, rec, flags, lds_bytes);
  }
  if (block && n_docs > n_big) {
    NgRest* rest = ng_rest(ex, n_docs);
    if (prof)
      hipLaunchKernelGGL((k_gr_ngrams<256, true>), dim3((uint32_t)(n_docs - n_big)), dim3(64 * kNgWaves), 0, stream,
                         (const DevStage*)stage, gr_step, perm, ndocs, ex, n_big, rest, rec, prof);
    else
      hipLaunchKernelGGL((k_gr_ngrams<256, false>), dim3((uint32_t)(n_docs - n_big)), dim3(64 * kNgWaves), 0,
                         stream, (const DevStage*)stage, gr_step, perm, ndocs, ex, n_big, rest, rec, nullptr);
    hipLaunchKernelGGL(k_gr_ngrams_rest, dim3(512), dim3(64), 0, stream, (const DevStage*)stage, gr_step, perm,
                       ndocs, ex, rest, pw, pw_n, t, rec, flags);
  }
  return (int)hipGetLastError();
}

int tb_stage_analyze_blk(hipStream_t stream, const void* plan, const void* stage, const uint8_t* bytes,
                         const int64_t* off, const int32_t* perm, int32_t nblocks, int32_t ndocs, char* scratch,
                         const int64_t* scratch_off, const uint64_t* pw, uint32_t pw_n, const uint16_t* s1,
                         const uint32_t* s2, const uint16_t* l1, const int32_t* l2, int64_t* rec, uint32_t* flags,
                         uint32_t lds_bytes, uint64_t* prof, const uint8_t* dead, void* gr_export, int32_t n_split,
                         uint32_t split_bytes, int32_t threads, uint32_t* line_stats, const void* pre,
                         int32_t n_pre, const int64_t* dict_moff, const uint32_t* dict_bits, const uint32_t* dict_words) {
  if (nblocks <= 0) return 0;
  if (!perm || lds_bytes > kMaxLdsPerBlk || n_split < 0 || n_split > nblocks) return (int)hipErrorInvalidValue;
  if (threads != kBlockThreads) return (int)hipErrorInvalidValue;
  if (pre && (threads != kBlockThreads || n_pre != nblocks)) return (int)hipErrorInvalidValue;
  DevTables t{s1, s2, l1, l2};
  auto kern = pre ? k_stage_analyze_blk_pre : k_stage_analyze_blk;
  if (lds_bytes > 65536)
    (void)hipFuncSetAttribute((const void*)kern, hipFuncAttributeMaxDynamicSharedMemorySize, (int)lds_bytes);
  hipLaunchKernelGGL(kern, dim3(nblocks), dim3(threads), lds_bytes, stream,
                     (const DevPlan*)plan, (const DevStage*)stage, bytes, off, perm, ndocs, scratch, scratch_off, pw,
                     pw_n, t, rec, flags, lds_bytes, prof, dead, (GrExport*)gr_export, n_split,
                     split_bytes, line_stats, (const PreDoc*)pre, n_pre, DictIn{dict_moff, dict_bits, dict_words});
  return (int)hipGetLastError();
}

int tb_gr_dup_split(hipStream_t stream, const void* stage, int32_t gr_step, const int32_t* perm, int32_t n_split,
                    int32_t n_tasks, int32_t ndocs, const void* gr_export, const uint64_t* pw, uint32_t pw_n,
                    const uint16_t* s1, const uint32_t* s2, const uint16_t* l1, const int32_t* l2, int64_t* rec,
                    uint32_t* flags, uint32_t lds_bytes, uint32_t* cursor) {
  if (n_split <= 0 || n_tasks <= 0) return 0;
  if (!perm || !gr_export || gr_step < 0 || gr_step >= kMaxStageSteps || n_tasks > 2 * kMaxNgramEntries + 2 ||
      lds_bytes > kMaxLdsPerBlk)
    return (int)hipErrorInvalidValue;
  if (!cursor) return (int)hipErrorInvalidValue;
  DevTables t{s1, s2, l1, l2};
  if (lds_bytes > 65536)
    (void)hipFuncSetAttribute((const void*)k_gr_dup_split, hipFuncAttributeMaxDynamicSharedMemorySize, (int)lds_bytes);
  const int cus = device_cus();
  int per_cu = 0;
  if (hipOccupancyMaxActiveBlocksPerMultiprocessor(&per_cu, (const void*)k_gr_dup_split, kBlockThreads, lds_bytes) !=
          hipSuccess || per_cu <= 0)
    per_cu = 1;
  const int64_t total = (int64_t)n_split * n_tasks;
  const int grid = (int)std::min<int64_t>(total, (int64_t)cus * per_cu);
  (void)hipMemsetAsync(cursor, 0, sizeof(uint32_t), stream);
  hipLaunchKernelGGL(k_gr_dup_split, dim3((uint32_t)grid), dim3(kBlockThreads), lds_bytes, stream,
                     (const DevStage*)stage, gr_step, perm, n_split, n_tasks, ndocs, (const GrExport*)gr_export, pw,
                     pw_n, t, rec, flags, lds_bytes, cursor);
  return (int)hipGetLastError();
}

// ... 96 lines not shown
                     WT, w_scale, bias, rec, width, prof);
  return (int)hipGetLastError();
}

int tb_c4_pass_a(hipStream_t stream, const void* c4, const uint8_t* bytes, const int64_t* off, const int32_t* perm,
                 int32_t ndocs, char* scratch, const int64_t* scratch_off, const uint64_t* pw, uint32_t pw_n,
                 const uint16_t* s1, const uint32_t* s2, const uint16_t* l1, const int32_t* l2, int64_t* rec,
                 int64_t* src, uint32_t* flags, uint32_t lds_bytes, uint64_t* prof, int32_t nblocks,
                 const uint8_t* dead, const uint32_t* line_stats, uint32_t* c4_words, const int64_t* dict_loff,
                 const uint32_t* dict_ldata) {
  if (ndocs <= 0) return 0;
  if (nblocks <= 0) nblocks = ndocs;
  if (lds_bytes > kMaxLdsPerDoc) return (int)hipErrorInvalidValue;
  DevTables t{s1, s2, l1, l2};
  if (lds_bytes > 65536)
    (void)hipFuncSetAttribute((const void*)k_c4_pass_a, hipFuncAttributeMaxDynamicSharedMemorySize, (int)lds_bytes);
  hipLaunchKernelGGL(k_c4_pass_a, dim3(nblocks), dim3(64), lds_bytes, stream, (const DevC4*)c4, bytes, off, perm, ndocs,
                     scratch, scratch_off, pw, pw_n, t, rec, src, flags, lds_bytes, prof, dead, line_stats, c4_words,
                     DictLines{dict_loff, dict_ldata});
  return (int)hipGetLastError();
}

int tb_c4_pass_b(hipStream_t stream, const uint8_t* bytes, const int64_t* off, int32_t ndocs, const char* scratch,
                 const int64_t* scratch_off, const int64_t* src, const int64_t* new_off, uint8_t* out) {
  if (ndocs <= 0) return 0;
  hipLaunchKernelGGL(k_c4_pass_b, dim3(ndocs), dim3(256), 0, stream, bytes, off, ndocs, scratch, scratch_off, src,
                     new_off, out);
  return (int)hipGetLastError();
}


int tb_gate(hipStream_t stream, const void* gate, const int64_t* const* recs, int32_t nrecs, int32_t ndocs,
            const uint32_t* flags, uint8_t* dead, int32_t code) {
  if (ndocs <= 0) return 0;
  if (nrecs < 0 || nrecs > kMaxGateSteps || code <= 0 || code > 255) return (int)hipErrorInvalidValue;
  GateRecs r{};
  for (int i = 0; i < nrecs; ++i) r.p[i] = recs[i];
  hipLaunchKernelGGL(k_gate, dim3((ndocs + 255) / 256), dim3(256), 0, stream, (const DevGate*)gate, r, ndocs, flags,
                     dead, (uint8_t)code);
  return (int)hipGetLastError();
}

size_t tb_sizeof_gate() { return sizeof(DevGate); }

int tb_resolve(hipStream_t stream, const void* rp, const int64_t* const* recs, int32_t nrecs, int32_t ndocs,
               const uint32_t* flags, const uint8_t* const* vb, const int64_t* const* vo, int32_t nver,
               int32_t* fail, uint8_t* status, uint8_t* fver, int64_t* lanes, int64_t* sc, uint8_t* out,
               int64_t cap, int64_t* out_off, int32_t* rows, int32_t* err) {
  if (ndocs <= 0) return 0;
  if (nrecs < 0 || nrecs > kMaxGateSteps || nver < 1 || nver > kMaxVersions) return (int)hipErrorInvalidValue;
  GateRecs r{};
  for (int i = 0; i < nrecs; ++i) r.p[i] = recs[i];
  VersionTab vt{};
  for (int i = 0; i < nver; ++i) {
    vt.b[i] = vb[i];
    vt.off[i] = vo[i];
  }
  hipLaunchKernelGGL(k_resolve, dim3((ndocs + 255) / 256), dim3(256), 0, stream, (const DevResolve*)rp, r, ndocs,
                     flags, vt, fail, status, fver, lanes);
  for (int j = 0; j < 4; ++j) {
    const int rc = tb_scan_strided_i64(stream, lanes + j, 4, ndocs, sc + (int64_t)j * ndocs);
    if (rc) return rc;
  }
  if (cap / (ndocs > 0 ? ndocs : 1) > 8192)
    hipLaunchKernelGGL(k_compact<256>, dim3(ndocs), dim3(kCompactThreads), 0, stream, status, fver, vt, ndocs, sc, out, cap, out_off, rows,
                     err);
  else
    hipLaunchKernelGGL(k_compact<64>, dim3((ndocs + 3) / 4), dim3(kCompactThreads), 0, stream, status, fver, vt, ndocs, sc, out, cap, out_off, rows,
                     err);
  return (int)hipGetLastError();
}

size_t tb_sizeof_resolve() { return sizeof(DevResolve); }


int tb_pow_table(hipStream_t stream, uint64_t* pw, uint32_t n) {
  hipLaunchKernelGGL(k_pow_table, dim3((n + 256) / 256), dim3(256), 0, stream, pw, n);
  return (int)hipGetLastError();
}

int tb_phase_slots() { return kPhaseSlots; }
int tb_stage_waves() { return TB_STAGE_WPE; }

int tb_abi_version() { return 24; }
size_t tb_sizeof_plan() { return sizeof(DevPlan); }
size_t tb_sizeof_stage() { return sizeof(DevStage); }
size_t tb_sizeof_c4() { return sizeof(DevC4); }

}
```

csrc/host/devplan_build.cpp:

```cpp
#include "devplan_build.h"

#include <algorithm>
#include <array>
#include <atomic>
#include <cmath>
#include <cstring>
#include <stdexcept>

#include "../common/docproc.h"

namespace tb {

int dev_kind_of(const StepCfg& c) {
  switch (c.kind) {
    case StepKind::GopherQuality: return DK_GOPHER_QUALITY;
    case StepKind::GopherRepetition: return DK_GOPHER_REP;
    case StepKind::FineWebQuality: return DK_FINEWEB;
    case StepKind::LanguageDetection: return DK_LANGID;
    default: return DK_NONE;
  }
}

bool device_supported(const StepCfg& c, std::string* why) {
  if (c.kind == StepKind::GopherRepetition) {
// ... 233 lines not shown
    if (k > 0 && entries[k][0] <= entries[k - 1][0]) throw std::invalid_argument("resolve: steps out of order");
    if (c4_version[k] >= kMaxVersions || (c4_version[k] >= 0 && rp.gate.steps[k].kind != GK_C4))
      throw std::invalid_argument("resolve: content version out of range");
    rp.step_index[k] = entries[k][0];
    rp.c4_version[k] = c4_version[k];
  }
  return rp;
}

void resolve_host(const DevResolve& rp, const std::vector<const int64_t*>& recs, int64_t ndocs,
                  const uint32_t* flags, const std::vector<const char*>& vdata,
                  const std::vector<const int64_t*>& voff, std::vector<int32_t>& fail, std::vector<uint8_t>& status,
                  std::string& out, std::vector<int64_t>& out_off, std::vector<int32_t>& rows) {
  for (int s = 0; s < rp.gate.n_steps; ++s) {
    if (rp.gate.steps[s].slot < 0 || rp.gate.steps[s].slot >= (int)recs.size())
      throw std::runtime_error("resolve record slot out of range");
    if (rp.c4_version[s] >= (int)voff.size()) throw std::runtime_error("resolve version out of range");
  }
  fail.assign(ndocs, -1);
  status.assign(ndocs, 0);
  std::vector<int32_t> ver(ndocs, 0);
  for (int64_t doc = 0; doc < ndocs; ++doc)
    resolve_doc(rp, recs.data(), ndocs, doc, flags ? flags[doc] : 0u, fail[doc], status[doc], ver[doc]);
  out.clear();
  out_off.assign(ndocs + 1, 0);
  rows.assign(ndocs, 0);
  int64_t pos = 0;
  for (uint8_t want : {kResolveKept, kResolveFiltered})
    for (int64_t doc = 0; doc < ndocs; ++doc) {
      if (status[doc] != want) continue;
      const int v = ver[doc];
      out_off[pos] = (int64_t)out.size();
      rows[pos++] = (int32_t)doc;
      out.append(vdata[v] + voff[v][doc], (size_t)(voff[v][doc + 1] - voff[v][doc]));
    }
  out_off[pos] = (int64_t)out.size();
}

std::vector<uint64_t> pow_table(uint32_t n) {
  std::vector<uint64_t> pw(2 * (size_t)n + 2);
  pw[0] = 1;
  pw[n + 1] = 1;
  for (uint32_t i = 1; i <= n; ++i) {
    pw[i] = hmul(pw[i - 1], kHashBase);
    pw[n + 1 + i] = hmul(pw[n + i], kHashBaseInv);
  }
  return pw;
}

uint64_t scratch_bytes_for(uint32_t doc_len, bool split) { return scratch_bytes_for_dev(doc_len, split); }

static std::atomic<uint64_t> g_scratch_need_milli{0};
static std::atomic<uint64_t> g_scratch_need_len{0};
static void note_scratch(uint64_t peak, uint32_t n) {
  const uint64_t over = peak > 4096 ? peak - 4096 : 0;
  const uint64_t m = over * 1000 / ((uint64_t)n + 64);
  uint64_t cur = g_scratch_need_milli.load(std::memory_order_relaxed);
  while (m > cur && !g_scratch_need_milli.compare_exchange_weak(cur, m)) {}
  if (m >= cur) g_scratch_need_len.store(n, std::memory_order_relaxed);
}
static std::atomic<bool> g_scratch_probe{false};
void set_scratch_probe(bool on) { g_scratch_probe = on; }
static uint64_t emu_cap(uint32_t n, bool split) {
  return g_scratch_probe ? 1024 * ((uint64_t)n + 64) + 4096 : scratch_bytes_for(n, split);
}
std::pair<double, uint32_t> scratch_need(bool reset) {
  const std::pair<double, uint32_t> r{g_scratch_need_milli.load() / 1000.0, (uint32_t)g_scratch_need_len.load()};
  if (reset) { g_scratch_need_milli = 0; g_scratch_need_len = 0; }
  return r;
}

uint64_t line_stats_buffer_words(const int64_t* off, int64_t ndocs) { return line_stats_words(off, ndocs); }

void emulate_stage(const std::vector<StepCfg>& steps, const std::vector<int>& idx, int64_t ndocs,
                   const char* data, const int64_t* off, int nthreads, const LangidModel* lid,
                   std::vector<int64_t>& rec, std::vector<uint32_t>& flags, uint32_t lds_bytes, const uint8_t* dead,
                   bool weak_keys, uint32_t* line_stats, int split_tasks, DictIn dict) {
  DevPlan* plan = new DevPlan();
  std::memset(plan, 0, sizeof(DevPlan));
  DevStage st = build_stage(steps, idx, *plan);
  int gr_pos = -1;
  for (int s = 0; s < st.n_steps; ++s)
    if (st.steps[s].kind == DK_GOPHER_REP) gr_pos = s;
  bool has_lid = false;
  for (int s = 0; s < st.n_steps; ++s) has_lid |= st.steps[s].kind == DK_LANGID;
  if (has_lid && !lid) { delete plan; throw std::runtime_error("language model required"); }
  rec.assign((size_t)st.width_total * ndocs, 0);
  flags.assign(ndocs, 0);
  uint32_t maxlen = 0;
  for (int64_t i = 0; i < ndocs; ++i) maxlen = std::max<uint32_t>(maxlen, (uint32_t)(off[i + 1] - off[i]));
  std::vector<uint64_t> pw = pow_table(maxlen + 16);
  const UcdView ucd = host_ucd();
  parallel_for(ndocs, nthreads, [&](int64_t a, int64_t b) {
    std::vector<char> scratch;
    std::vector<char> lds(lds_bytes + 16);
    for (int64_t i = a; i < b; ++i) {
      if (dead && dead[i]) continue;
      const uint32_t n = (uint32_t)(off[i + 1] - off[i]);
      const uint64_t need = emu_cap(n, split_tasks > 0 && gr_pos >= 0);
      if (scratch.size() < need) scratch.resize(need);
      DocCtx<SeqPar> x;
      x.ucd = ucd;
      x.pw = pw.data();
      x.pw_n = (uint32_t)(pw.size() / 2 - 1);
      x.ipw = pw.data() + x.pw_n + 1;
      x.scr = scratch.data();
      x.cap = need;
      x.lds = lds_bytes ? lds.data() : nullptr;
      x.lcap = lds_bytes;
      x.flag = &flags[i];
      x.weak_keys = weak_keys;
      StageOut out{rec.data(), (uint32_t)ndocs, (uint32_t)i};
      out.dict = dict;
      if (line_stats) out.line_stats = line_stats + line_stats_base(off[i], i);
      GrExport ex{};
      if (split_tasks > 0 && gr_pos >= 0) out.gr_export = &ex;
      analyze_stage(x, st, *plan, lid ? lid->tables() : LidTables{}, (const uint8_t*)data + off[i], n, out);
      if (x.overflow) continue;
      if (!out.gr_export || !ex.valid) {
        note_scratch(x.peak, n);
        continue;
      }
      const DevStep& ds = st.steps[gr_pos];
      int64_t* r = rec.data() + (int64_t)ds.rec_prefix * ndocs + i * ds.width;
      const uint64_t region = (ex.free_cap / (uint64_t)split_tasks) & ~255ull;
      uint64_t task_peak = 0;
      bool over = false;
      for (int t = 0; t < split_tasks; ++t) {
        DocCtx<SeqPar> y;
        y.ucd = ucd;
        y.pw = pw.data();
        y.pw_n = x.pw_n;
        y.ipw = x.ipw;
        y.scr = ex.free_base + (uint64_t)t * region;
        y.cap = region;
        y.lds = lds_bytes ? lds.data() : nullptr;
        y.lcap = lds_bytes;
        y.flag = &flags[i];
        if (t < ds.n_dup) gr_dup_one_order(y, ds, t, ex, r);
        else if (t < ds.n_dup + ds.n_top) gr_top_one_order(y, ds, t - ds.n_dup, ex, r);
        else if (t < ds.n_dup + ds.n_top + 2) gr_lines_split(y, t - ds.n_dup - ds.n_top, ex, r);
        if (y.overflow) { y.set_flag(DOC_NEEDS_CPU | DOC_OVERFLOW); over = true; }
        task_peak = std::max<uint64_t>(task_peak, (y.peak + 255) & ~255ull);
      }
      if (!over) note_scratch((uint64_t)(ex.free_base - scratch.data()) + (uint64_t)split_tasks * task_peak, n);
    }
  });
  delete plan;
}


void emulate_c4(const StepCfg& step, int64_t ndocs, const char* data, const int64_t* off, int nthreads,
                std::vector<int64_t>& rec, std::string& new_data, std::vector<int64_t>& new_off,
                std::vector<uint32_t>& flags, uint32_t lds_bytes, const uint8_t* dead, const uint32_t* line_stats,
                uint32_t* c4_words, DictLines dict_lines) {
  DevC4 c4 = build_c4(step);
  rec.assign((size_t)rec::C4_WIDTH * ndocs, 0);
  flags.assign(ndocs, 0);
  std::vector<std::string> outs(ndocs);
  uint32_t maxlen = 0;
  for (int64_t i = 0; i < ndocs; ++i) maxlen = std::max<uint32_t>(maxlen, (uint32_t)(off[i + 1] - off[i]));
  std::vector<uint64_t> pw = pow_table(maxlen + 16);
  const UcdView ucd = host_ucd();
  parallel_for(ndocs, nthreads, [&](int64_t a, int64_t b) {
    std::vector<char> scratch;
    std::vector<char> lds(lds_bytes + 16);
    for (int64_t i = a; i < b; ++i) {
      if (dead && dead[i]) continue;
      const uint32_t n = (uint32_t)(off[i + 1] - off[i]);
      const uint64_t need = emu_cap(n, false);
      if (scratch.size() < need) scratch.resize(need);
      DocCtx<SeqPar> x;
      x.ucd = ucd;
      x.pw = pw.data();
      x.pw_n = (uint32_t)(pw.size() / 2 - 1);
      x.ipw = pw.data() + x.pw_n + 1;
      x.scr = scratch.data();
      x.cap = need;
      x.lds = lds_bytes ? lds.data() : nullptr;
      x.lcap = lds_bytes;
      x.flag = &flags[i];
      int64_t src[2] = {-1, 0};
      const uint8_t* b = (const uint8_t*)data + off[i];
      c4_pass_a(x, c4, b, n, rec.data() + i * rec::C4_WIDTH, src,
                line_stats ? line_stats + line_stats_base(off[i], i) : nullptr, c4_words ? c4_words + i : nullptr,
                dict_lines.at((uint32_t)i));
      if (!x.overflow) note_scratch(x.peak, n);
      if (flags[i] & DOC_NEEDS_CPU) continue;
      if (src[0] < 0) outs[i].assign((const char*)b, n);
      else outs[i].assign(scratch.data() + src[0], (size_t)src[1]);
    }
  });
  new_off.assign(ndocs + 1, 0);
  size_t tot = 0;
  for (auto& s : outs) tot += s.size();
  new_data.clear();
  new_data.reserve(tot);
  for (int64_t i = 0; i < ndocs; ++i) {
    new_data += outs[i];
    new_off[i + 1] = (int64_t)new_data.size();
// ... 5 lines not shown
```

csrc/host/module.cpp:

```cpp
#include <pybind11/numpy.h>
#include <pybind11/pybind11.h>
#include <pybind11/stl.h>

#include <cstring>
#include <optional>
#include <thread>
#include <unordered_map>

#include "../common/badwords.h"
#include "../common/bpe.h"
#include "../common/bpe_classes.inc"
#include "../common/langid.h"
#include "../common/ucd_tables.inc"
#include "filters.h"
#include "html.h"
#include "html_entities.inc"
#include "json.h"
#include "pipeline.h"
#include "devplan_build.h"
#include "rustfmt.h"
#include "text.h"

namespace py = pybind11;
using namespace tb;
// ... 730 lines not shown
  m.def("device_supported", [](const StepCfg& c) {
    std::string why;
    bool ok = device_supported(c, &why);
    return py::make_tuple(ok, why);
  });
  m.def("build_device_plan", [](const std::vector<StepCfg>& steps, const std::vector<std::vector<int>>& stages) {
    auto plan = std::make_unique<DevPlan>();
    std::memset(plan.get(), 0, sizeof(DevPlan));
    py::list st;
    for (auto& idx : stages) {
      DevStage d = build_stage(steps, idx, *plan);
      st.append(py::bytes((const char*)&d, sizeof(d)));
    }
    return py::make_tuple(py::bytes((const char*)plan.get(), sizeof(DevPlan)), st);
  });
  m.def("build_c4", [](const StepCfg& c) {
    DevC4 d = build_c4(c);
    return py::bytes((const char*)&d, sizeof(d));
  });
  m.def("build_gate", [](const std::vector<StepCfg>& steps, const std::vector<std::array<int, 3>>& entries) {
    DevGate g = build_gate(steps, entries);
    return py::bytes((const char*)&g, sizeof(g));
  });
  m.def("gate_fails", [](const StepCfg& c, const std::vector<int64_t>& r) {
    if ((int)r.size() < record_width(c)) throw std::runtime_error("record too short");
    DevGateStep g = build_gate_step(c, 0, 0);
    return gate_fails(g, r.data());
  });
  m.def("decide_status", [](const StepCfg& c, const std::vector<int64_t>& r) {
    if ((int)r.size() < record_width(c)) throw std::runtime_error("record too short");
    return (int)decide_status(c, r.data());
  });
  m.attr("SIZEOF_DEV_GATE") = sizeof(DevGate);
  m.attr("SIZEOF_DEV_RESOLVE") = sizeof(DevResolve);
  m.attr("MAX_VERSIONS") = kMaxVersions;
  m.def("build_resolve", [](const std::vector<StepCfg>& steps, const std::vector<std::array<int, 3>>& entries,
                            const std::vector<int>& c4_version) {
    DevResolve rp = build_resolve(steps, entries, c4_version);
    return py::bytes((const char*)&rp, sizeof(rp));
  });
  m.def("resolve_host", [](const py::bytes& blob, const std::vector<py::array_t<int64_t, py::array::c_style>>& recs,
                           int64_t ndocs, py::array_t<uint32_t, py::array::c_style> flags,
                           const std::vector<py::array_t<uint8_t, py::array::c_style>>& vdata,
                           const std::vector<py::array_t<int64_t, py::array::c_style>>& voff) {
    std::string bs = blob;
    if (bs.size() != sizeof(DevResolve)) throw std::runtime_error("bad resolve blob");
    DevResolve rp;
    std::memcpy(&rp, bs.data(), sizeof(rp));
    if ((int64_t)flags.size() < ndocs || vdata.size() != voff.size()) throw std::runtime_error("resolve: operand shapes");
    for (int s = 0; s < rp.gate.n_steps; ++s) {
      const DevGateStep& st = rp.gate.steps[s];
      if (st.slot < 0 || st.slot >= (int)recs.size() ||
          (int64_t)recs[st.slot].size() < ((int64_t)st.prefix + st.width) * ndocs)
        throw std::runtime_error("resolve record buffer too short");
    }
    std::vector<const int64_t*> rp_ptrs;
    for (auto& r : recs) rp_ptrs.push_back(r.data());
    std::vector<const char*> vd;
    std::vector<const int64_t*> vo;
    for (size_t v = 0; v < vdata.size(); ++v) {
      if ((int64_t)voff[v].size() != ndocs + 1) throw std::runtime_error("resolve: version offsets length");
      vd.push_back((const char*)vdata[v].data());
      vo.push_back(voff[v].data());
    }
    std::vector<int32_t> fail, rows;
    std::vector<uint8_t> status;
    std::string out;
    std::vector<int64_t> out_off;
    {
      py::gil_scoped_release nogil;
      resolve_host(rp, rp_ptrs, ndocs, flags.data(), vd, vo, fail, status, out, out_off, rows);
    }
    return py::make_tuple(to_numpy(std::move(fail)), to_numpy(std::move(status)), str_to_numpy(std::move(out)),
                          to_numpy(std::move(out_off)), to_numpy(std::move(rows)));
  });
  m.def("stage_layout", [](const py::bytes& b) {
    std::string s = b;
    DevStage d;
    std::memcpy(&d, s.data(), sizeof(d));
    py::list out;
    for (int i = 0; i < d.n_steps; ++i) out.append(py::make_tuple(d.steps[i].kind, d.steps[i].width, d.steps[i].rec_prefix));
    return py::make_tuple(d.width_total, out);
  });
  m.def("pow_table", [](uint32_t n) { return to_numpy(pow_table(n)); });
  m.def("scratch_bytes_for", [](uint32_t n, bool split) { return scratch_bytes_for(n, split); }, py::arg("n"),
        py::arg("split") = false);
  m.def("scratch_need", [](bool reset) { return scratch_need(reset); }, py::arg("reset") = false);
  m.def("set_scratch_probe", &set_scratch_probe);
  m.attr("SCRATCH_PER_BYTE") = kScratchPerByte;
  m.attr("SCRATCH_PER_BYTE_SPLIT") = kScratchPerByteSplit;
  m.attr("C4_MAX_GROWTH") = kC4MaxGrowth;
  m.attr("SIZEOF_DEV_PLAN") = sizeof(DevPlan);
  m.attr("SIZEOF_DEV_STAGE") = sizeof(DevStage);
  m.attr("SIZEOF_DEV_C4") = sizeof(DevC4);
  m.attr("OFFSETOF_REC_BASE") = offsetof(DevStep, rec_base);
  m.attr("SIZEOF_DEV_STEP") = sizeof(DevStep);
  m.attr("OFFSETOF_STEPS") = offsetof(DevStage, steps);
  m.def("emulate_stage", [](const std::vector<StepCfg>& steps, const std::vector<int>& idx,
                            py::array_t<uint8_t, py::array::c_style> data, py::array_t<int64_t, py::array::c_style> off,
                            int nthreads, std::shared_ptr<LangidModel> lid, uint32_t lds_bytes,
                            std::optional<py::array_t<uint8_t, py::array::c_style>> dead, bool weak_keys,
                            std::optional<py::array_t<uint32_t, py::array::c_style>> line_stats, int split_tasks,
                            std::optional<py::array_t<int64_t, py::array::c_style>> dict_moff,
                            std::optional<py::array_t<uint32_t, py::array::c_style>> dict_bits,
                            std::optional<py::array_t<uint32_t, py::array::c_style>> dict_words) {
    std::vector<int64_t> rec;
    std::vector<uint32_t> flags;
    const int64_t nd = (int64_t)off.size() - 1;
    if (dead && (int64_t)dead->size() < nd) throw std::runtime_error("dead mask too short");
    const uint8_t* dp = dead ? dead->data() : nullptr;
    uint32_t* lp = nullptr;
    if (line_stats) {
      if ((uint64_t)line_stats->size() < line_stats_buffer_words(off.data(), nd)) throw std::runtime_error("line_stats too short");
      lp = line_stats->mutable_data();
    }
    DictIn dict;
    if (dict_moff) {
      if ((int64_t)dict_moff->size() < nd || !dict_bits) throw std::runtime_error("dict marks: operand shapes");
      const int64_t* mo = dict_moff->data();
      for (int64_t d = 0; d < nd; ++d) {
        if (mo[d] < 0) continue;
        uint32_t C = 0;
        for (int64_t i = off.data()[d]; i < off.data()[d + 1]; ++i) C += (data.data()[i] & 0xC0) != 0x80;
        if (mo[d] + (int64_t)(2 * (((C + 1 + 63) / 64) * 2)) > (int64_t)dict_bits->size())
          throw std::runtime_error("dict marks: bitmap out of range");
      }
      dict.moff = mo;
      dict.bits = dict_bits->data();
    }
    if (dict_words) {
      if ((int64_t)dict_words->size() < nd) throw std::runtime_error("dict words: operand shapes");
      dict.words = dict_words->data();
    }
    {
      py::gil_scoped_release nogil;
      emulate_stage(steps, idx, nd, (const char*)data.data(), off.data(), nthreads, lid.get(), rec, flags, lds_bytes,
                    dp, weak_keys, lp, split_tasks, dict);
    }
    return py::make_tuple(to_numpy(std::move(rec)), to_numpy(std::move(flags)));
  }, py::arg("steps"), py::arg("idx"), py::arg("data"), py::arg("offsets"), py::arg("nthreads") = 8,
     py::arg("lid") = nullptr, py::arg("lds_bytes") = 0, py::arg("dead") = py::none(),
     py::arg("weak_keys") = false, py::arg("line_stats") = py::none(), py::arg("split_tasks") = 0,
     py::arg("dict_moff") = py::none(), py::arg("dict_bits") = py::none(), py::arg("dict_words") = py::none());
  m.def("line_stats_words", [](py::array_t<int64_t, py::array::c_style> off) {
    return line_stats_buffer_words(off.data(), (int64_t)off.size() - 1);
  }, "u32 words of a batch's C4 line export buffer (docproc.h line_stats_base)");
  m.def("gate_host", [](const py::bytes& gate, const std::vector<py::array_t<int64_t, py::array::c_style>>& recs,
                        int64_t ndocs, py::array_t<uint32_t, py::array::c_style> flags,
                        py::array_t<uint8_t, py::array::c_style> dead, int code) {
    std::string gs = gate;
    if (gs.size() != sizeof(DevGate)) throw std::runtime_error("bad gate blob");
    if (code <= 0 || code > 255) throw std::runtime_error("gate code out of range");
    if ((int64_t)dead.size() < ndocs || (int64_t)flags.size() < ndocs) throw std::runtime_error("gate: operand shapes");
    DevGate g;
    std::memcpy(&g, gs.data(), sizeof(g));
    std::vector<const int64_t*> rp;
    for (int s = 0; s < g.n_steps; ++s) {
      const DevGateStep& st = g.steps[s];
      if (st.kind == GK_NONE) continue;
      if (st.slot < 0 || st.slot >= (int)recs.size()) throw std::runtime_error("gate slot out of range");
      if ((int64_t)recs[st.slot].size() < ((int64_t)st.prefix + st.width) * ndocs)
        throw std::runtime_error("gate record buffer too short");
    }
    for (auto& r : recs) rp.push_back(r.data());
    gate_host(g, rp, ndocs, flags.data(), dead.mutable_data(), (uint8_t)code);
  });
// ... 46 lines not shown
```

textblaster_amd/ops/kernels.py:

```python
from __future__ import annotations

import ctypes
from typing import Optional

import numpy as np

from ..errors import DeviceError

_P = ctypes.c_void_p
_I32 = ctypes.c_int32
_U32 = ctypes.c_uint32
_I64 = ctypes.c_int64
_SZ = ctypes.c_size_t

ABI_VERSION = 24

_SIGS = {
    "tb_stage_analyze": [_P, _P, _P, _P, _P, _P, _I32, _P, _P, _P, _U32, _P, _P, _P, _P, _P, _P, _U32, _P, _I32, _I32, _P,
                         _P, _P, _P, _P, _P],
    "tb_gr_split_wave": [_P, _P, _I32, _P, _I32, _I32, _I32, _P, _P, _U32, _P, _P, _P, _P, _P, _P, _U32, _I32, _P,
                         _I32],
    "tb_c4_pass_a": [_P, _P, _P, _P, _P, _I32, _P, _P, _P, _U32, _P, _P, _P, _P, _P, _P, _P, _U32, _P, _I32, _P, _P,
                     _P, _P, _P],
    "tb_stage_analyze_blk": [_P, _P, _P, _P, _P, _P, _I32, _I32, _P, _P, _P, _U32, _P, _P, _P, _P, _P, _P,
                             _U32, _P, _P, _P, _I32, _U32, _I32, _P, _P, _I32, _P, _P, _P],
    "tb_sizeof_pre_doc": [],
    "tb_pre_decode": [_P, _P, _P, _P, _I32, _P, _P, _U32, _P, _P, _P, _P, _P],
    "tb_gr_dup_split": [_P, _P, _I32, _P, _I32, _I32, _I32, _P, _P, _U32, _P, _P, _P, _P, _P, _P, _U32, _P],
    "tb_sizeof_gr_export": [],
    "tb_c4_pass_a_blk": [_P, _P, _P, _P, _P, _I32, _I32, _P, _P, _P, _U32, _P, _P, _P, _P, _P, _P, _P, _U32, _P, _P,
                         _P, _P, _P, _P],
    "tb_gate": [_P, _P, _P, _I32, _I32, _P, _P, _I32],
    "tb_sizeof_gate": [],
    "tb_resolve": [_P, _P, _P, _I32, _I32, _P, _P, _P, _I32, _P, _P, _P, _P, _P, _P, _I64, _P, _P, _P],
    "tb_sizeof_resolve": [],
    "tb_block_threads": [],
    "tb_badwords_match": [_P, _P, _P, _I32, _P, _P, _I32, _I32, _P, _U32, _P, _U32, _P, _P, _P, _P, _P, _P, _P, _P, _P,
                          _U32],
    "tb_langid_mfma": [_P, _P, _P, _P, _I32, _P, _P, _P, _P, _P, _P, _P, ctypes.c_double, _P, _P, _I32, _P],
    "tb_langid_prepare": [_P, _P, _P],
    "tb_pre_wcanon": [_P, _P, _P, _P, _I32, _P, _P, _U32, _P, _U32, _P],
    "tb_langid_aux_bytes": [],
    "tb_c4_pass_b": [_P, _P, _P, _I32, _P, _P, _P, _P, _P],
    "tb_pow_table": [_P, _P, _U32],
    "tb_html_sizes": [_P, _P, _P, _I32, _P, _P, _P, _P, _I32, _P, _U32, _P],
    "tb_html_scatter": [_P, _P, _P, _I32, _P, _P, _P, _P, _I32, _P, _U32, _P, _P],
    "tb_bpe_count": [_P, _P, _P, _P, _P, _I32, _P],
    "tb_sizeof_bpe": [],
    "tb_abi_version": [],
    "tbrt_device_count": [_P], "tbrt_set_device": [_I32], "tbrt_get_device": [_P], "tbrt_device_sync": [],
    "tbrt_mem_info": [_P, _P], "tbrt_malloc": [_P, _SZ], "tbrt_free": [_P], "tbrt_host_alloc": [_P, _SZ],
    "tbrt_host_free": [_P], "tbrt_empty_cache": [], "tbrt_cache_stats": [_P], "tbrt_stream_create": [_P, _I32],
    "tbrt_stream_destroy": [_P], "tbrt_stream_sync": [_P], "tbrt_stream_priority_range": [_P, _P],
    "tbrt_event_create": [_P, _I32], "tbrt_event_destroy": [_P], "tbrt_event_record": [_P, _P],
    "tbrt_event_sync": [_P], "tbrt_event_query": [_P], "tbrt_event_elapsed": [_P, _P, _P],
    "tbrt_stream_wait_event": [_P, _P], "tbrt_memcpy_h2d": [_P, _P, _SZ, _P], "tbrt_memcpy_d2h": [_P, _P, _SZ, _P],
    "tbrt_memcpy_d2d": [_P, _P, _SZ, _P], "tbrt_memset": [_P, _I32, _SZ, _P],
    "tb_scan_strided_i64": [_P, _P, _I64, _I64, _P],
    "tb_phase_slots": [],
    "tb_stage_waves": [],
    "tb_sizeof_plan": [],
    "tb_sizeof_stage": [],
    "tb_sizeof_c4": [],
}


def _dict_ptrs(dict_in):
    if dict_in is None:
        return 0, 0, 0
    return tuple(_ptr(a) for a in dict_in)


PRE_DOC = np.dtype([("off", "<u8"), ("prop", "<u8"), ("wbm", "<u8"), ("nl_pos", "<u8"), ("nl_len", "<u8"),
                    ("n", "<u4"), ("C", "<u4"), ("dict", "<u4"), ("NL", "<u4"), ("tcs", "<u4"), ("tce", "<u4"),
                    ("nl_a", "<u4"), ("nl_e", "<u4"), ("wtmp", "<u8"), ("wcs", "<u8"), ("wce", "<u8"),
                    ("wbs", "<u8"), ("wbe", "<u8"), ("wal", "<u8"), ("W", "<u4"), ("pad", "<u4"),
                    ("wh", "<u8"), ("wtab", "<u8"), ("wk", "<u8"), ("wpb", "<u8"), ("wcsum", "<u8"),
                    ("wslot", "<u8"), ("wid", "<u8"), ("wl", "<u8"), ("wready", "<u4"), ("pad2", "<u4")])
PRE_WCHUNK = 2048
PRE_TILE = 16384


class DevBpe(ctypes.Structure):
    _fields_ = [("byte_id", _P), ("keys", _P), ("vals", _P), ("cls1", _P), ("cls2", _P), ("added", _P),
                ("mask", _U32), ("n_added", _I32), ("added_off", _I32 * 9), ("post_add", _I32)]


class BpeTables:

    def __init__(self, spec, cls_tables):
        from . import hiprt

        self.arrays = [hiprt.to_device(a) for a in (spec.byte_id, spec.keys, spec.vals, cls_tables[0], cls_tables[1],
                                                    spec.added)]
        if len(spec.added_off) > 9:
            raise DeviceError("bpe: too many added tokens")
        st = DevBpe()
        st.byte_id, st.keys, st.vals, st.cls1, st.cls2, st.added = [a.data_ptr() for a in self.arrays]
        st.mask = spec.mask
        st.n_added = max(len(spec.added_off) - 1, 0)
        for i, v in enumerate(spec.added_off):
            st.added_off[i] = v
        st.post_add = spec.post_add
        self.struct = st


def declare(lib: ctypes.CDLL) -> None:
    for name, args in _SIGS.items():
        fn = getattr(lib, name)
        fn.argtypes = args
        fn.restype = ctypes.c_size_t if name.startswith("tb_sizeof") else ctypes.c_int


def _ptr(t) -> Optional[int]:
    return None if t is None else t.data_ptr()


def _check(rc: int, what: str) -> None:
    if rc != 0:
        raise DeviceError(f"{what} failed with hipError_t {rc}")


class Kernels:

    def __init__(self, device: int):
        from .. import native
        from . import hiprt

        self.device = device
        self.lib = native.hip()
        h = native.host()
        if self.lib.tb_abi_version() != ABI_VERSION:
            raise DeviceError(f"libtbhip.so ABI {self.lib.tb_abi_version()} != {ABI_VERSION}; rebuild")
        if (self.lib.tb_sizeof_plan() != h.SIZEOF_DEV_PLAN or self.lib.tb_sizeof_stage() != h.SIZEOF_DEV_STAGE
                or self.lib.tb_sizeof_gate() != h.SIZEOF_DEV_GATE
                or self.lib.tb_sizeof_resolve() != h.SIZEOF_DEV_RESOLVE):
            raise DeviceError("libtbhip.so and _tbhost disagree on the device plan layout; rebuild")
        self.sizeof_gr_export = int(self.lib.tb_sizeof_gr_export())
        if int(self.lib.tb_sizeof_pre_doc()) != PRE_DOC.itemsize:
            raise DeviceError("libtbhip.so and ops/kernels.py disagree on PreDoc; rebuild")
        s1, s2, l1, l2 = h.ucd_tables()
        self.tabs = [hiprt.to_device(a) for a in (s1, s2, l1, l2)]
        self._pw = None
        self._pw_n = 0

    @staticmethod
    def stream() -> int:
        from . import hiprt

        return hiprt.current_stream().handle

    def pow_table(self, n: int):
        if n > self._pw_n:
            from . import hiprt

            cap = max(n, 1 << 16)
            cap = 1 << (cap - 1).bit_length()
            self._pw = hiprt.empty(2 * cap + 2, np.int64)
            _check(self.lib.tb_pow_table(self.stream(), self._pw.data_ptr(), cap), "tb_pow_table")
            hiprt.current_stream().synchronize()
            self._pw_n = cap
        return self._pw, self._pw_n

    def stage_analyze(self, plan, stage, bytes_, off, perm, ndocs, scratch, scratch_off, pw, pw_n, rec, flags,
                      lds_bytes=0, prof=None, waves=0, nblocks=0, dead=None, line_stats=None, gr_export=None,
                      dict_in=None):
        t = self.tabs
        if gr_export is not None and gr_export.nbytes < max(nblocks, 0) * self.sizeof_gr_export:
            raise DeviceError("stage_analyze: export buffer too small")
        rc = self.lib.tb_stage_analyze(
            self.stream(), plan.data_ptr(), stage.data_ptr(), bytes_.data_ptr(), off.data_ptr(), _ptr(perm), ndocs,
            scratch.data_ptr(), scratch_off.data_ptr(), pw.data_ptr(), pw_n, t[0].data_ptr(), t[1].data_ptr(),
            t[2].data_ptr(), t[3].data_ptr(), rec.data_ptr(), flags.data_ptr(), lds_bytes, _ptr(prof), waves, nblocks,
            _ptr(dead), _ptr(line_stats), _ptr(gr_export), *_dict_ptrs(dict_in))
        _check(rc, "tb_stage_analyze")

    def gr_export_wave_bytes(self, n_docs: int) -> int:
        return n_docs * self.sizeof_gr_export + 16 + 4 * n_docs

    def gr_split_wave(self, stage, gr_step, perm, n_docs, n_tasks, ndocs, gr_export, pw, pw_n, rec, flags, lds_bytes,
                      block=True, prof=None, n_big=0):
        if not 0 <= n_big <= n_docs:
            raise DeviceError("gr_split_wave: n_big out of range")
        if gr_export.nbytes < self.gr_export_wave_bytes(n_docs) or perm.numel() < n_docs:
            raise DeviceError("gr_split_wave: operand shapes")
        t = self.tabs
        rc = self.lib.tb_gr_split_wave(self.stream(), stage.data_ptr(), gr_step, perm.data_ptr(), n_docs, n_tasks,
                                       ndocs, gr_export.data_ptr(), pw.data_ptr(), pw_n, t[0].data_ptr(),
                                       t[1].data_ptr(), t[2].data_ptr(), t[3].data_ptr(), rec.data_ptr(),
                                       flags.data_ptr(), lds_bytes, 1 if block else 0, _ptr(prof), int(n_big))
        _check(rc, "tb_gr_split_wave")

    def stage_analyze_blk(self, plan, stage, bytes_, off, perm_long, nlong, ndocs, scratch, scratch_off, pw, pw_n,
                          rec, flags, lds_bytes=0, prof=None, dead=None, gr_export=None, n_split=0, split_bytes=0,
                          threads=512, line_stats=None, pre=None, n_pre=0, dict_in=None):
        t = self.tabs
        if gr_export is not None and gr_export.nbytes < n_split * self.sizeof_gr_export:
            raise DeviceError("stage_analyze_blk: export buffer too small")
        if not 0 <= n_split <= nlong:
            raise DeviceError("stage_analyze_blk: n_split out of range")
        rc = self.lib.tb_stage_analyze_blk(
            self.stream(), plan.data_ptr(), stage.data_ptr(), bytes_.data_ptr(), off.data_ptr(), perm_long.data_ptr(),
            nlong, ndocs, scratch.data_ptr(), scratch_off.data_ptr(), pw.data_ptr(), pw_n, t[0].data_ptr(),
            t[1].data_ptr(), t[2].data_ptr(), t[3].data_ptr(), rec.data_ptr(), flags.data_ptr(), lds_bytes, _ptr(prof),
            _ptr(dead), _ptr(gr_export), n_split if gr_export is not None else 0, split_bytes, int(threads),
            _ptr(line_stats), _ptr(pre), int(n_pre) if pre is not None else 0, *_dict_ptrs(dict_in))
        _check(rc, "tb_stage_analyze_blk")

    def pre_decode(self, bytes_, off, perm_pre, npre, dead, pre, tiles_max, cnt):
        if perm_pre.numel() < npre or cnt.numel() < npre * tiles_max or pre.nbytes < npre * PRE_DOC.itemsize:
            raise DeviceError("pre_decode: operand shapes")
        t = self.tabs
        rc = self.lib.tb_pre_decode(self.stream(), bytes_.data_ptr(), off.data_ptr(), perm_pre.data_ptr(), npre,
                                    _ptr(dead), pre.data_ptr(), int(tiles_max), cnt.data_ptr(), t[0].data_ptr(),
                                    t[1].data_ptr(), t[2].data_ptr(), t[3].data_ptr())
        _check(rc, "tb_pre_decode")

    def pre_wcanon(self, bytes_, off, perm_pre, npre, dead, pre, chunks_max, pw, pw_n, flags):
        if perm_pre.numel() < npre or pre.nbytes < npre * PRE_DOC.itemsize or chunks_max <= 0:
            raise DeviceError("pre_wcanon: operand shapes")
        rc = self.lib.tb_pre_wcanon(self.stream(), bytes_.data_ptr(), off.data_ptr(), perm_pre.data_ptr(), npre,
                                    _ptr(dead), pre.data_ptr(), int(chunks_max), pw.data_ptr(), pw_n,
                                    flags.data_ptr())
        _check(rc, "tb_pre_wcanon")

    def gr_dup_split(self, stage, gr_step, perm, n_split, n_tasks, ndocs, gr_export, pw, pw_n, rec, flags, lds_bytes,
                     cursor):
        if gr_export.nbytes < n_split * self.sizeof_gr_export or perm.numel() < n_split or cursor.nbytes < 4:
            raise DeviceError("gr_dup_split: operand shapes")
        t = self.tabs
        rc = self.lib.tb_gr_dup_split(self.stream(), stage.data_ptr(), gr_step, perm.data_ptr(), n_split, n_tasks, ndocs,
                                      gr_export.data_ptr(), pw.data_ptr(), pw_n, t[0].data_ptr(), t[1].data_ptr(),
                                      t[2].data_ptr(), t[3].data_ptr(), rec.data_ptr(), flags.data_ptr(), lds_bytes,
                                      cursor.data_ptr())
        _check(rc, "tb_gr_dup_split")

    def c4_pass_a_blk(self, c4, bytes_, off, perm_long, nlong, ndocs, scratch, scratch_off, pw, pw_n, rec, src, flags,
                      lds_bytes=0, prof=None, dead=None, line_stats=None, c4_words=None, dict_lines=None):
        t = self.tabs
        dl = dict_lines or (None, None)
        rc = self.lib.tb_c4_pass_a_blk(
            self.stream(), c4.data_ptr(), bytes_.data_ptr(), off.data_ptr(), perm_long.data_ptr(), nlong, ndocs,
            scratch.data_ptr(), scratch_off.data_ptr(), pw.data_ptr(), pw_n, t[0].data_ptr(), t[1].data_ptr(),
            t[2].data_ptr(), t[3].data_ptr(), rec.data_ptr(), src.data_ptr(), flags.data_ptr(), lds_bytes, _ptr(prof),
            _ptr(dead), _ptr(line_stats), _ptr(c4_words), _ptr(dl[0]), _ptr(dl[1]))
        _check(rc, "tb_c4_pass_a_blk")

    def badwords_match(self, bytes_, off, ndocs, table, fold, matched, root=None, cjk=None, root0=-1, cjk0=0,
                       dead=None, dead_max=0, seg_bytes=2048, seg_doc=None, seg_idx=None):
        t = self.tabs
        f1, f2 = fold
        slots = table.numel() // 4
        if slots < 1 or slots & (slots - 1) or matched.numel() < ndocs or off.numel() < ndocs + 1:
            raise DeviceError("badwords_match: operand shapes")
        for a in (root, cjk, dead):
            if a is not None and a.numel() < ndocs:
                raise DeviceError("badwords_match: per-document array shorter than the batch")
        if (seg_doc is None) != (seg_idx is None) or (seg_doc is not None and seg_doc.numel() != seg_idx.numel()):
# ... 98 lines not shown
```

textblaster_amd/pipeline/device.py:

```python
from __future__ import annotations

import dataclasses
from typing import Dict, List, Optional, Tuple

import numpy as np

from .. import native
from ..errors import DeviceError
from ..ops.kernels import PRE_DOC, PRE_TILE, PRE_WCHUNK
from ..utils import metrics, tracing
from .plan import ExecPlan
from . import tuning
from .tuning import DeviceTuning

SCRATCH_ALIGN = 256


@dataclasses.dataclass
class DeviceResult:
    stage_recs: List[np.ndarray]
    c4_recs: Dict[int, np.ndarray]
    versions: Dict[int, Tuple[np.ndarray, np.ndarray]]
    flags: np.ndarray
    timings: Dict[str, float]
# ... 272 lines not shown
    return passes, pass_of_step, gates


BW_SEG_BYTES = 2048


def bw_segments(lens: np.ndarray, growth: int, seg: int):
    bound = lens.astype(np.int64) + int(growth)
    extra = np.maximum((bound + seg - 1) // seg - 1, 0)
    idx = np.nonzero(extra)[0]
    if not len(idx):
        z = np.zeros(0, dtype=np.int32)
        return z, z
    cnt = extra[idx]
    seg_doc = np.repeat(idx, cnt).astype(np.int32)
    starts = np.cumsum(cnt) - cnt
    seg_idx = (np.arange(int(cnt.sum()), dtype=np.int64) - np.repeat(starts, cnt) + 1).astype(np.int32)
    return seg_doc, seg_idx


def bw_dead_max(plan: ExecPlan, passes, pass_of_step: Dict[int, int]) -> Dict[int, int]:
    out = {}
    for sp in plan.steps:
        if sp.type != "C4BadWordsFilter":
            continue
        later = [p for j, p in pass_of_step.items() if j > sp.index]
        out[sp.index] = min(later) if later else len(passes)
    return out


class DeviceRunner:
    N_SLOTS = 2

    def __init__(self, steps_native, plan: ExecPlan, device, langid=None, max_batch_bytes: int = 384 << 20,
                 token_counters=None, slots: Optional[int] = None, host_threads: int = 8,
                 tune: Optional[DeviceTuning] = None):
        from ..ops import hiprt

        self.tune = tu = (tune or tuning.from_env()).replace(slots=slots or None)
        self.rt = hiprt
        hiprt.set_blocking_events(tu.event_blocking)
        self.host_threads = max(1, int(host_threads))
        self.dict_marks = dict_marks_wanted(plan, steps_native, tu)
        with tracing.trace_range("tb.init.hip_context"):
            self.device = hiprt.parse_device(device)
            if self.device >= hiprt.device_count():
                raise DeviceError(f"no HIP device {self.device}")
            hiprt.set_device(self.device)
        self.plan = plan
        self.steps = steps_native
        h = native.host()
        blk_prio = tu.blk_priority
        self.stream_layout = tu.streams
        if tu.slots:
            self.N_SLOTS = max(1, int(tu.slots))
        else:
            try:
                _, total = hiprt.mem_info()
            except Exception:
                total = 0
            per_slot = int(1.25 * 176 * max_batch_bytes) + (2 << 30)
            self.N_SLOTS = 3 if total >= 3 * per_slot + (8 << 30) else 2
        self.slots = [_Slot() for _ in range(self.N_SLOTS)]
        if self.stream_layout == "serial":
            one = hiprt.Stream()
            for sl in self.slots:
                sl.main = sl.s_lid = sl.s_blk = sl.s_c4 = sl.s_c4blk = sl.s_h2d = sl.s_d2h = one
        else:
            h2d, d2h = hiprt.Stream(), hiprt.Stream()
            for sl in self.slots:
                sl.main = sl.s_c4 = hiprt.Stream()
                sl.s_blk = sl.s_lid = sl.s_c4blk = hiprt.Stream(priority=blk_prio)
                sl.s_h2d, sl.s_d2h = h2d, d2h
        init = self.slots[0].main
        with hiprt.stream(init):
            from ..ops.kernels import Kernels

            with tracing.trace_range("tb.init.kernels"):
                self.k = Kernels(self.device)
            plan_b, stage_bs = h.build_device_plan(steps_native, plan.stages)
            self.plan_t = self._to_dev(plan_b)
            self.stage_ts = [self._to_dev(b) for b in stage_bs]
            self.stage_layout = [h.stage_layout(b) for b in stage_bs]
            self.c4_ts = {i: self._to_dev(h.build_c4(steps_native[i])) for i in plan.c4_steps}
            self.has_lid = any(steps_native[i].kind == h.StepKind.LanguageDetection
                               for st in plan.stages for i in st)
            self.lid_b = self.lid_E = self.lid_WT = None
            self.lid_w_scale = 0.0
            if self.has_lid:
                if langid is None:
                    raise DeviceError("LanguageDetectionFilter needs a language-id model")
                self.lid_b = hiprt.to_device(np.ascontiguousarray(langid.b, dtype=np.float32))
                self.lid_E = hiprt.to_device((langid.E.astype(np.int16) + 128).astype(np.uint8))
                self.lid_aux = self.k.langid_prepare(self.lid_E)
                self.lid_WT = hiprt.to_device(np.ascontiguousarray(langid.head_bf16_t()).reshape(-1))
                self.lid_w_scale = float(langid.w_scale)
            self.c4_growth = int(h.C4_MAX_GROWTH)
            self.gating = tu.gate
            self.passes, self.pass_of_step, gates = plan_passes(
                plan, self.stage_layout, steps_native, self.gating, tu.lid_gate and self.has_lid)
            self.gate_ts = {p: self._to_dev(b) for p, (b, _) in gates.items()}
            self.bw_dead_max = bw_dead_max(plan, self.passes, self.pass_of_step)
            self.gate_need = {p: need for p, (_, need) in gates.items()}
            self.resolve_t = None
            if tu.device_resolve:
                blob = build_resolve(plan, self.stage_layout, steps_native)
                if blob is not None:
                    self.resolve_t = self._to_dev(blob)
                    self.resolve_need = [w for w, _ in self.stage_layout] + [7] * len(plan.c4_steps)
            self.bpe = []
            if self.resolve_t is not None and tu.device_tokens:
                self.bpe = [(i, self.k.bpe_tables(sp)) for i, sp in (token_counters or [])]
            with tracing.trace_range("tb.init.pow_table"):
                self.k.pow_table(1 << 22)
            init.synchronize()
        self.stage_waves = int(self.k.lib.tb_stage_waves())
        self.lds_bytes = tu.lds_bytes or (163840 // (4 * self.stage_waves)) & ~255
        self.lds_bytes_c4 = tu.lds_bytes_c4
        self.long_doc_bytes = tu.long_doc_bytes
        self.lds_bytes_blk = tu.lds_bytes_blk
        self.block_threads = int(self.k.lib.tb_block_threads())
        self.lds_bytes_dup = tu.lds_bytes_dup or self.lds_bytes_blk
        self.split_doc_bytes = tu.split_doc_bytes
        if self.split_doc_bytes > 0:
            self.split_doc_bytes = max(self.split_doc_bytes, self.long_doc_bytes)
        self.pre_doc_bytes = tu.pre_doc_bytes
        self.pre_wcanon = tu.pre_wcanon
        if self.pre_doc_bytes > 0:
            self.pre_doc_bytes = max(self.pre_doc_bytes, 65536, self.long_doc_bytes)
        self.gr_split = {}
        for si, idx in enumerate(plan.stages):
            grs = [k for k, (kind, _, _) in enumerate(self.stage_layout[si][1]) if kind == KIND_GOPHER_REP]
            if len(grs) == 1:
                st = steps_native[idx[grs[0]]]
                if st.n_dup + st.n_top > 0:
                    self.gr_split[si] = (grs[0], st.n_dup + st.n_top + 2)
        self.line_stats_stage = line_stats_stages(plan, self.stage_layout, tu)
        self.scratch_rates = (max(int(h.SCRATCH_PER_BYTE), tu.scratch_rate[0]),
                              max(int(h.SCRATCH_PER_BYTE_SPLIT), tu.scratch_rate[1]))
        self.lds_bytes_split = tu.lds_bytes_split
        self.ngram_block = tu.ngram_block
        self.ngram_big_bytes = tu.ngram_big_bytes
        self.zero_copy = tu.zero_copy
        self.phase_prof = tu.phase_prof
        self.phase_totals: Dict[str, np.ndarray] = {}
        self.phase_docs: Dict[str, int] = {}
        self.copy_threads = tu.copy_threads
        self._next_slot = 0
        self._bw_table = None
        self._bw_fold = None

    def bind_thread(self) -> None:
        self.rt.set_device(self.device)

    def synchronize(self) -> None:
        self.rt.synchronize()

    def _bw_tables(self, bw: BwInput):
        rt = self.rt
        if self._bw_fold is None:
            f1, f2 = native.host().ucd_fold_tables()
            self._bw_fold = (rt.to_device(f1), rt.to_device(f2))
        if self._bw_table is None or self._bw_table[0] != bw.gen:
            self._bw_table = (bw.gen, rt.to_device(np.ascontiguousarray(bw.table, dtype=np.uint32)))
        return self._bw_table[1], self._bw_fold

# ... 267 lines not shown
                lstats = rt.empty(4 * (vlen // 8 + 16 * ndocs) + 16, np.uint32)
                keep.append(lstats)
            for s, sv in enumerate(self.plan.stage_version):
                if sv != ver:
                    continue
                width_total, layout = self.stage_layout[s]
                rec = rt.zeros(width_total * ndocs, np.int64)
                lid_at = [(width, prefix) for kind, width, prefix in layout if kind == KIND_LANGID]
                ev_pre = self._record(main)
                keep.append(ev_pre)
                ev_lid = ev_blk = None
                prof = self._prof_buf(ndocs, keep, f"stage{s}")
                lid_pass = ("lid", s) in self.passes
                if lid_pass:
                    slot.s_lid.wait_event(ev_pre)
                    with rt.stream(slot.s_lid):
                        with self._ktimed(keep, "langid"):
                            for width, prefix in lid_at:
                                self._langid(vb, vo, d_perm, ndocs, scratch, d_soff, rec[prefix * ndocs:], width,
                                             flags, self._prof_buf(ndocs, keep, f"langid{s}"))
                        if pass_idx in self.gate_ts:
                            self.k.gate(self.gate_ts[pass_idx], [rec], ndocs, flags, dead, pass_idx + 1, 0,
                                        self.gate_need[pass_idx])
                        ev_pre = self._record(slot.s_lid)
                        keep.append(ev_pre)
                    main.wait_event(ev_pre)
                    pass_idx += 1
                skip = dead if pass_idx > 0 else None
                ls_out = lstats if self.line_stats_stage.get(ver) == s else None
                if n_long:
                    slot.s_blk.wait_event(ev_pre)
                    n_split, gx = 0, None
                    if s in self.gr_split and self.split_doc_bytes > 0:
                        huge = np.nonzero(lens[perm[:n_long]] > self.split_doc_bytes)[0]
                        if len(huge):
                            n_split = int(huge[-1]) + 1
                            gx = rt.zeros(n_split * self.k.sizeof_gr_export, np.uint8, slot.s_blk)
                            keep.append(gx)
                    esz = self.k.sizeof_gr_export
                    with rt.stream(slot.s_blk), self._ktimed(keep, f"stage{s}_blk"):
                        if ver == 0 and pre_v0 is None:
                            pre_v0 = self._pre_decode(vb, vo, d_perm, lens[perm[:n_long]], skip, keep, flags,
                                                      self.pre_wcanon)
                        pre, n_pre = pre_v0 if ver == 0 else (None, 0)
                        bt = self.block_threads
                        segs = ((0, n_pre, bt, True), (n_pre, n_long, bt, False))
                        for a0, a1, thr, with_pre in segs:
                            if a1 <= a0:
                                continue
                            ns = max(0, min(n_split, a1) - a0)
                            self.k.stage_analyze_blk(self.plan_t, self.stage_ts[s], vb, vo, d_perm[a0:a1], a1 - a0,
                                                     ndocs, scratch, d_soff[a0:], pw, pw_n, rec, flags,
                                                     self.lds_bytes_blk, prof, skip,
                                                     gx[a0 * esz:] if (gx is not None and ns) else None, ns,
                                                     self.split_doc_bytes, thr, ls_out,
                                                     pre if with_pre else None, a1 - a0 if with_pre else 0,
                                                     dict_in.get(ver))
                        if n_split:
                            gr_pos, n_tasks = self.gr_split[s]
                            cur = rt.empty(1, np.uint32)
                            keep.append(cur)
                            self.k.gr_dup_split(self.stage_ts[s], gr_pos, d_perm[:n_split], n_split, n_tasks, ndocs,
                                                gx, pw, pw_n, rec, flags, self.lds_bytes_dup, cur)
                        ev_blk = self._record(slot.s_blk)
                        keep.append(ev_blk)
                if lid_at and not lid_pass:
                    slot.s_lid.wait_event(ev_pre)
                    with rt.stream(slot.s_lid), self._ktimed(keep, "langid"):
                        for width, prefix in lid_at:
                            self._langid(vb, vo, d_perm, ndocs, scratch, d_soff, rec[prefix * ndocs:], width,
                                         flags, self._prof_buf(ndocs, keep, f"langid{s}"))
                        ev_lid = self._record(slot.s_lid)
                        keep.append(ev_lid)
                if n_long < ndocs:
                    nw = ndocs - n_long
                    gxw = None
                    if s in self.gr_split:
                        gxw = rt.zeros(self.k.gr_export_wave_bytes(nw), np.uint8)
                        keep.append(gxw)
                    with self._ktimed(keep, f"stage{s}"):
                        self.k.stage_analyze(self.plan_t, self.stage_ts[s], vb, vo, d_perm[n_long:], ndocs,
                                             scratch, d_soff[n_long:], pw, pw_n, rec, flags,
                                             self.lds_bytes, prof, self.stage_waves, nw, skip, ls_out, gxw,
                                             dict_in.get(ver))
                        if gxw is not None:
                            gr_pos, n_tasks = self.gr_split[s]
                            n_big = int(np.count_nonzero(lens_perm[n_long:] > self.ngram_big_bytes))
                            self.k.gr_split_wave(self.stage_ts[s], gr_pos, d_perm[n_long:], nw, n_tasks - 2, ndocs,
                                                 gxw, pw, pw_n, rec, flags, self.lds_bytes_split, self.ngram_block,
                                                 self._prof_buf(ndocs, keep, f"ngram{s}"), n_big)
                if ev_lid is not None:
                    main.wait_event(ev_lid)
                if ev_blk is not None:
                    main.wait_event(ev_blk)
                if pass_idx in self.gate_ts:
                    self.k.gate(self.gate_ts[pass_idx], [rec], ndocs, flags, dead, pass_idx + 1, 0,
                                        self.gate_need[pass_idx])
                pass_idx += 1
                stage_recs_d[s] = rec
            c4_here = [i for i in self.plan.c4_steps if self.plan.steps[i].version_in == ver]
            for i in c4_here:
                c4_scratch = scratch
                rec = rt.zeros(7 * ndocs, np.int64)
                src = rt.zeros(2 * ndocs, np.int64)
                new_off = rt.zeros(ndocs + 1, np.int64)
                c4w = None
                if self.dict_marks and ver in dict_in:
                    c4w = rt.empty(ndocs, np.uint32).fill_(0xFF)
                    keep.append(c4w)
                    dict_in[ver + 1] = (None, None, c4w)
                cap = vlen + self.c4_growth * ndocs + 16
                out = rt.empty(cap, np.uint8)
                ev_main = self._record(main)
                slot.s_c4.wait_event(ev_main)
                slot.s_c4.wait_event(ready[ver])
                keep.append(ev_main)
                skip = dead if pass_idx > 0 else None
                prof = self._prof_buf(ndocs, keep, f"c4_step{i}")
                ev_c4blk = None
                if n_long:
                    ev_c4 = self._record(slot.s_c4)
                    slot.s_c4blk.wait_event(ev_c4)
                    keep.append(ev_c4)
                    with rt.stream(slot.s_c4blk):
                        self.k.c4_pass_a_blk(self.c4_ts[i], vb, vo, d_perm[:n_long], n_long, ndocs, c4_scratch,
                                             d_soff, pw, pw_n, rec, src, flags, self.lds_bytes_blk, prof, skip,
                                             lstats, c4w, dict_lines.get(i))
                        ev_c4blk = self._record(slot.s_c4blk)
                        keep.append(ev_c4blk)
                with rt.stream(slot.s_c4), self._ktimed(keep, f"c4_step{i}"):
                    if n_long < ndocs:
                        self.k.c4_pass_a(self.c4_ts[i], vb, vo, d_perm[n_long:], ndocs, c4_scratch, d_soff[n_long:], pw,
                                         pw_n, rec, src, flags, self.lds_bytes_c4, prof, ndocs - n_long, skip,
                                         lstats, c4w, dict_lines.get(i))
                    if ev_c4blk is not None:
                        slot.s_c4.wait_event(ev_c4blk)
                    rt.scan_strided_i64(src[1:], 2, ndocs, new_off[1:])
                    self.k.c4_pass_b(vb, vo, ndocs, c4_scratch, d_soff, src, new_off, out)
                    if pass_idx in self.gate_ts:
                        self.k.gate(self.gate_ts[pass_idx], [rec], ndocs, flags, dead, pass_idx + 1, 0,
                                        self.gate_need[pass_idx])
                    ev = self._record(slot.s_c4)
                pass_idx += 1
                versions[ver + 1] = (out, new_off, cap)
                ready[ver + 1] = ev
                tails.append(ev)
                c4_recs_d[i] = rec
                keep.append(src)
        for ev in tails:
            main.wait_event(ev)
        bw_d = {}
        for i in sorted(bw):
            x = bw[i]
            sp = self.plan.steps[i]
            vb, vo, _ = versions[sp.version_in]
            table, fold = self._bw_tables(x)
            m = rt.empty(max(ndocs, 1), np.int8)
            v = sp.version_in
            with self._ktimed(keep, "badwords"):
                self.k.badwords_match(vb, vo, ndocs, table, fold, m, bw_dev.get((i, "root")), bw_dev.get((i, "cjk")),
                                      x.root0, x.cjk0, dead, self.bw_dead_max[i], BW_SEG_BYTES,
                                      bw_dev.get((v, "seg_doc")), bw_dev.get((v, "seg_idx")))
            keep += [table, m]
            bw_d[i] = m
        res_d = None
        if self.resolve_t is not None:
            recs = [r for r in stage_recs_d] + [c4_recs_d[i] for i in self.plan.c4_steps]
# ... 172 lines not shown
```

Before: 13.20 million.

## Specialize stage kernels per step mix and split GopherQuality word stats into separate kernel

Adds compile-time specialized variants of the stage-analysis kernel (GR+GQ, GR-only, FW-only), selected per stage from its step kinds. This is meant to cut dead code paths and register pressure in the generic kernel. For stages with one GopherRepetition and one GopherQuality step, the word-level GQ statistics are moved out. The GR step exports the word spans, and a separate k_gq_wave kernel computes word and byte counts by walking raw UTF-8 bytes instead of codepoint props. The cost is an extra launch, export-buffer traffic, and slower byte-level codepoint walks for the Sigma-casing and stop-word paths. It also fixes an out-of-bounds read in the 2-byte ASCII fast path.

```diff
diff --git a/csrc/common/devplan.h b/csrc/common/devplan.h
--- a/csrc/common/devplan.h
+++ b/csrc/common/devplan.h
@@ -73,6 +73,24 @@
   DevStep steps[kMaxStageSteps];
 };
 
+enum : uint32_t { SK_GQ = 1, SK_GR = 2, SK_FW = 4, SK_LID = 8, SK_ALL = 15, SK_GQ_EXT = 16 };
+enum StageVariant : int32_t { SV_GENERIC = 0, SV_GR_GQX = 1, SV_GR = 2, SV_FW = 3, SV_COUNT = 4 };
+TB_HD int32_t stage_variant(const DevStage& st) {
+  int n_gq = 0, n_gr = 0, n_fw = 0, n_other = 0, gr_orders = 0;
+  for (int s = 0; s < st.n_steps; ++s) {
+    const DevStep& d = st.steps[s];
+    if (d.kind == DK_GOPHER_QUALITY) ++n_gq;
+    else if (d.kind == DK_GOPHER_REP) { ++n_gr; gr_orders = d.n_top + d.n_dup; }
+    else if (d.kind == DK_FINEWEB) ++n_fw;
+    else if (d.kind != DK_LANGID) ++n_other;
+  }
+  if (n_other) return SV_GENERIC;
+  if (n_gr == 1 && n_gq == 1 && n_fw == 0 && gr_orders > 0) return SV_GR_GQX;
+  if (n_gr >= 1 && n_gq == 0 && n_fw == 0) return SV_GR;
+  if (n_fw >= 1 && n_gq == 0 && n_gr == 0) return SV_FW;
+  return SV_GENERIC;
+}
+
 constexpr int kMaxStopSets = 4;
 
 struct DevPlan {
diff --git a/csrc/common/docproc.h b/csrc/common/docproc.h
--- a/csrc/common/docproc.h
+++ b/csrc/common/docproc.h
@@ -57,6 +57,29 @@
   TB_HD uint32_t cp(uint32_t i) const {
     int len;
     return utf8_decode(b, o(i), nb, &len);
+  }
+  TB_HD uint32_t next(uint32_t i) const { return i + 1; }
+  TB_HD uint32_t prev(uint32_t i) const { return i - 1; }
+};
+
+struct ByteCps {
+  const uint8_t* b = nullptr;
+  uint32_t nb = 0;
+  UcdView ucd;
+  TB_HD uint32_t cp(uint32_t i) const {
+    int len;
+    return utf8_decode(b, i, nb, &len);
+  }
+  TB_HD uint32_t p(uint32_t i) const { return compact_prop(ucd.props(cp(i))); }
+  TB_HD uint32_t next(uint32_t i) const {
+    ++i;
+    while (i < nb && !utf8_is_lead(b[i])) ++i;
+    return i;
+  }
+  TB_HD uint32_t prev(uint32_t i) const {
+    --i;
+    while (i > 0 && !utf8_is_lead(b[i])) --i;
+    return i;
   }
 };
 
@@ -291,7 +314,7 @@
       [&](uint32_t i, uint32_t k, int&) {
         uint16_t cpk;
         const uint32_t c0 = b[i];
-        if (asc && (c0 < 0x80 || (c0 & 0xFEu) == 0xC2u)) {
+        if (asc && (c0 < 0x80 || ((c0 & 0xFEu) == 0xC2u && i + 1 < n))) {
           cpk = asc[c0 < 0x80 ? c0 : (((c0 & 0x1Fu) << 6) | (b[i + 1] & 0x3Fu))];
         } else {
           int len;
@@ -820,23 +843,23 @@
   x.reset(mark);
 }
 
-template <class F>
-TB_HD void lower_bytes(const UcdView& ucd, const Cps& cv, uint32_t s, uint32_t e, F&& push) {
+template <class CV, class F>
+TB_HD void lower_bytes(const UcdView& ucd, const CV& cv, uint32_t s, uint32_t e, F&& push) {
   uint8_t buf[4];
-  const PropArr prop = cv.props();
-  for (uint32_t k = s; k < e; ++k) {
+  for (uint32_t k = s; k < e; k = cv.next(k)) {
     uint32_t c = cv.cp(k);
     uint32_t lc;
     if (c == 0x3A3) {
       bool before = false, after = false;
-      for (uint32_t j = k; j > s; --j) {
-        uint32_t p = prop[j - 1];
+      for (uint32_t j = k; j > s;) {
+        j = cv.prev(j);
+        uint32_t p = cv.p(j);
         if (p & P16_CASE_IGN) continue;
         before = (p & P_CASED) != 0;
         break;
       }
-      for (uint32_t j = k + 1; j < e; ++j) {
-        uint32_t p = prop[j];
+      for (uint32_t j = cv.next(k); j < e; j = cv.next(j)) {
+        uint32_t p = cv.p(j);
         if (p & P16_CASE_IGN) continue;
         after = (p & P_CASED) != 0;
         break;
@@ -851,12 +874,13 @@
   }
 }
 
-TB_HD bool is_stop_word(const UcdView& ucd, const DevStopSet& ss, const Cps& cv, uint32_t s, uint32_t e,
+template <class CV>
+TB_HD bool is_stop_word(const UcdView& ucd, const DevStopSet& ss, const CV& cv, uint32_t s, uint32_t e, uint32_t nc,
                         uint32_t b0, uint32_t b1) {
-  if (ss.n == 0 || (int32_t)(e - s) > ss.max_len) return false;
+  if (ss.n == 0 || (int32_t)nc > ss.max_len) return false;
   if (ss.lite_nslots > 0) {
     const uint32_t nb = b1 - b0;
-    if (nb <= 7u && nb == e - s) {
+    if (nb <= 7u && nb == nc) {
       uint64_t key = (uint64_t)nb << 56;
       for (uint32_t k = 0; k < nb; ++k) {
         uint32_t c = cv.b[b0 + k];
@@ -936,6 +960,11 @@
   PHView ph;
   uint32_t NR, NPR, tcs, tce;
   uint32_t lines_valid;
+  const uint32_t* cs;
+  const uint32_t* ce;
+  const uint8_t* alpha;
+  uint32_t gq_W;
+  uint32_t gq_valid;
 };
 
 TB_HD void gr_line_span(const uint32_t* rs, const uint32_t* rl, const OffArr& off, uint32_t tcs, uint32_t tce,
@@ -1182,11 +1211,18 @@
 TB_HD void gopher_rep_record(DocCtx<P>& x, const DevStep& ds, const uint8_t* b, const Cps& c,
                              const PHView& ph, const Words& w, int64_t* r, bool release_props = false,
                              GrExport* ex = nullptr, const PreDoc* pre = nullptr,
-                             const uint8_t* b_export = nullptr, Lines lines = Lines{}) {
+                             const uint8_t* b_export = nullptr, Lines lines = Lines{}, bool export_gq = false) {
   const uint32_t C = c.n;
   const PropArr prop = c.props();
   const OffArr off = c.offs();
   const int width = ds.width;
+  if (export_gq && ex) {
+    x.par.single([&]() {
+      ex->cs = w.cs; ex->ce = w.ce; ex->alpha = w.alpha; ex->bs = w.bs; ex->be = w.be;
+      ex->gq_W = w.n;
+      ex->gq_valid = 1u;
+    });
+  }
   uint32_t tcs, tce;
   trim_span(x, prop, C, tcs, tce);
   if (tcs >= tce) {
@@ -1767,8 +1803,8 @@
   return ~(((t & 0x7F7F7F7Fu) + 0x7F7F7F7Fu) | t | 0x7F7F7F7Fu);
 }
 
-template <class P>
-TB_HD uint64_t gq_byte_counts(DocCtx<P>& x, const uint8_t* b, uint32_t n) {
+template <class Par>
+TB_HD uint64_t gq_byte_counts(Par& par, const uint8_t* b, uint32_t n) {
   const uintptr_t a0 = (uintptr_t)b & ~(uintptr_t)3;
   const uint32_t head = (uint32_t)((uintptr_t)b - a0);
   const uint32_t nd = (head + n + 3) >> 2;
@@ -1784,7 +1820,7 @@
     }
     return v;
   };
-  return x.par.template sum<uint64_t>((nd + 3) >> 2, [&](uint32_t g) {
+  return par.template sum<uint64_t>((nd + 3) >> 2, [&](uint32_t g) {
     uint32_t d[6];
 #pragma unroll
     for (uint32_t i = 0; i < 6; ++i) d[i] = dw((int64_t)4 * g + i - 1);
@@ -1815,6 +1851,65 @@
       }
     }
     return acc;
+  });
+}
+
+template <class Par>
+TB_HD uint64_t gq_byte_counts_plain(Par& par, const uint8_t* b, uint32_t n) {
+  return par.template sum<uint64_t>(n, [&](uint32_t i) {
+    const uint32_t c0 = b[i];
+    if (c0 == '#') return (uint64_t)1 << 32;
+    if (c0 == 0xE2) return (uint64_t)(i + 2 < n && b[i + 1] == 0x80 && b[i + 2] == 0xA6);
+    if (c0 != '.' || (i > 0 && b[i - 1] == '.')) return (uint64_t)0;
+    uint32_t j = i;
+    while (j < n && b[j] == '.') ++j;
+    return (uint64_t)((j - i) / 3);
+  });
+}
+
+enum : uint32_t { GQF_CHARS = 1, GQF_ALPHA = 2, GQF_STOP = 4, GQF_ALL = 7 };
+template <class CV>
+TB_HD uint64_t gq_word_term(const UcdView& ucd, const DevStopSet& ss, const CV& cv, uint32_t s, uint32_t e,
+                            uint32_t nc, uint32_t b0, uint32_t b1, uint32_t al, uint32_t f) {
+  uint64_t v = 0;
+  if (f & GQF_CHARS) v |= (uint64_t)nc << 32;
+  if (f & GQF_ALPHA) v |= (uint64_t)al << 16;
+  if (f & GQF_STOP) v |= (uint64_t)is_stop_word(ucd, ss, cv, s, e, nc, b0, b1);
+  return v;
+}
+template <class Par, class TermF>
+TB_HD void gq_word_stats(Par& par, uint32_t W, TermF&& term, int64_t& sum_chars, int64_t& alpha, int64_t& stop) {
+  if (W < 65536u) {
+    const uint64_t as = par.template sum<uint64_t>(W, [&](uint32_t k) { return term(k, (uint32_t)GQF_ALL); });
+    sum_chars = (int64_t)(as >> 32);
+    alpha = (int64_t)((as >> 16) & 0xFFFFull);
+    stop = (int64_t)(as & 0xFFFFull);
+  } else {
+    sum_chars = par.template sum<int64_t>(W, [&](uint32_t k) { return (int64_t)(term(k, (uint32_t)GQF_CHARS) >> 32); });
+    alpha = par.template sum<int64_t>(W, [&](uint32_t k) { return (int64_t)(term(k, (uint32_t)GQF_ALPHA) >> 16); });
+    stop = par.template sum<int64_t>(W, [&](uint32_t k) { return (int64_t)term(k, (uint32_t)GQF_STOP); });
+  }
+}
+
+template <bool kSwar, class Par>
+TB_HD void gq_export_record(Par& par, const UcdView& ucd, const DevStopSet& ss, const GrExport& e,
+                            const uint8_t* b, uint32_t n, int64_t* r) {
+  const uint32_t W = e.gq_W;
+  ByteCps cv;
+  cv.b = b;
+  cv.nb = n;
+  cv.ucd = ucd;
+  const uint32_t *cs = e.cs, *ce = e.ce, *bs = e.bs, *be = e.be;
+  const uint8_t* al = e.alpha;
+  int64_t sum_chars = 0, alpha = 0, stop = 0;
+  gq_word_stats(par, W, [&](uint32_t k, uint32_t f) {
+    const uint32_t b0 = bs[k], b1 = be[k];
+    return gq_word_term(ucd, ss, cv, b0, b1, ce[k] - cs[k], b0, b1, (uint32_t)al[k], f);
+  }, sum_chars, alpha, stop);
+  const uint64_t he = kSwar ? gq_byte_counts(par, b, n) : gq_byte_counts_plain(par, b, n);
+  par.single([&]() {
+    r[0] = W; r[1] = sum_chars; r[2] = (int64_t)(he >> 32); r[3] = (int64_t)(he & 0xFFFFFFFFull);
+    r[7] = alpha; r[8] = stop;
   });
 }
 
@@ -2561,16 +2656,22 @@
 #endif
 constexpr bool kHotProps = TB_HOT_PROPS != 0;
 
-template <class P, bool kWithLid = true, bool kPre = false>
+template <class P, bool kWithLid = true, bool kPre = false, uint32_t kKinds = SK_ALL>
 TB_HD void analyze_stage(DocCtx<P>& x, const DevStage& st, const DevPlan& plan,
                          const LidTables& lid, const uint8_t* b, uint32_t n, StageOut& out) {
-  bool need_words = false, need_lines = false, need_ph = false, need_lid = false;
-  for (int s = 0; s < st.n_steps; ++s) {
-    const int k = st.steps[s].kind;
-    if (k == DK_GOPHER_QUALITY) need_words = need_lines = true;
-    if (k == DK_GOPHER_REP) need_words = need_ph = true;
-    if (k == DK_FINEWEB) need_words = need_lines = need_ph = true;
-    if (k == DK_LANGID) need_lid = true;
+  constexpr bool kGeneric = (kKinds & SK_ALL) == SK_ALL && !(kKinds & SK_GQ_EXT);
+  constexpr bool kGq = (kKinds & SK_GQ) != 0, kGr = (kKinds & SK_GR) != 0, kFw = (kKinds & SK_FW) != 0;
+  constexpr bool kGqExt = (kKinds & SK_GQ_EXT) != 0;
+  static_assert(!kGqExt || (kGq && kGr), "SK_GQ_EXT: GopherQuality next to the exporting GopherRepetition step");
+  bool need_words = kGq || kGr || kFw, need_lines = kGq || kFw, need_ph = kGr || kFw;
+  if constexpr (kGeneric) {
+    need_words = need_lines = need_ph = false;
+    for (int s = 0; s < st.n_steps; ++s) {
+      const int k = st.steps[s].kind;
+      if (k == DK_GOPHER_QUALITY) need_words = need_lines = true;
+      if (k == DK_GOPHER_REP) need_words = need_ph = true;
+      if (k == DK_FINEWEB) need_words = need_lines = need_ph = true;
+    }
   }
   x.stamp(PH_START);
   if (out.line_stats) x.par.single([&]() { out.line_stats[0] = kLineStatsNone; });
@@ -2592,9 +2693,12 @@
   const uint32_t* dict_marks = nullptr;
   uint32_t wfix = kNoWords;
   if (ndict && need_words) {
-    bool fw_only = true;
-    for (int s = 0; s < st.n_steps; ++s)
-      fw_only &= st.steps[s].kind != DK_GOPHER_QUALITY && st.steps[s].kind != DK_GOPHER_REP;
+    bool fw_only = !kGq && !kGr;
+    if constexpr (kGeneric) {
+      fw_only = true;
+      for (int s = 0; s < st.n_steps; ++s)
+        fw_only &= st.steps[s].kind != DK_GOPHER_QUALITY && st.steps[s].kind != DK_GOPHER_REP;
+    }
     if (!kPre) dict_marks = out.dict.marks(out.doc);
     if (!kPre && !dict_marks && fw_only) wfix = out.dict.nwords(out.doc);
     if (!dict_marks && wfix == kNoWords) {
@@ -2636,39 +2740,21 @@
     const DevStep& ds = st.steps[s];
     if ((so < st.n_steps) == (ds.kind == DK_GOPHER_REP)) continue;
     int64_t* r = out.rec + (int64_t)ds.rec_prefix * out.ndocs + (int64_t)out.doc * ds.width;
-    if (ds.kind == DK_GOPHER_QUALITY) {
-      const DevStopSet& ss = plan.stops[ds.stop_set];
-      const UcdView ucd = x.ucd;
+    if (kGq && ds.kind == DK_GOPHER_QUALITY) {
       auto lo32 = [](uint64_t v) { return (int64_t)(v & 0xFFFFFFFFull); };
       auto hi32 = [](uint64_t v) { return (int64_t)(v >> 32); };
-      int64_t sum_chars = 0;
-      const uint64_t as = x.par.template sum<uint64_t>(W, [&](uint32_t k) {
-        const uint32_t a = w.cs[k], e = w.ce[k];
-        return ((uint64_t)(e - a) << 32) | ((uint64_t)w.alpha[k] << 16) |
-               (uint64_t)is_stop_word(ucd, ss, c, a, e, w.bs[k], w.be[k]);
-      });
-      int64_t alpha, stop;
-      if (W < 65536u) {
-        sum_chars = hi32(as);
-        alpha = (int64_t)((as >> 16) & 0xFFFFull);
-        stop = (int64_t)(as & 0xFFFFull);
-      } else {
-        sum_chars = x.par.template sum<int64_t>(W, [&](uint32_t k) { return (int64_t)(w.ce[k] - w.cs[k]); });
-        alpha = x.par.template sum<int64_t>(W, [&](uint32_t k) { return (int64_t)w.alpha[k]; });
-        stop = x.par.template sum<int64_t>(W, [&](uint32_t k) {
-          return (int64_t)is_stop_word(ucd, ss, c, w.cs[k], w.ce[k], w.bs[k], w.be[k]);
-        });
-      }
-      x.stamp(PH_GQ_WORDS);
-      const uint64_t he = P::kWaves <= 1 ? gq_byte_counts(x, b, n) : x.par.template sum<uint64_t>(n, [&](uint32_t i) {
-        const uint32_t c0 = b[i];
-        if (c0 == '#') return (uint64_t)1 << 32;
-        if (c0 == 0xE2) return (uint64_t)(i + 2 < n && b[i + 1] == 0x80 && b[i + 2] == 0xA6);
-        if (c0 != '.' || (i > 0 && b[i - 1] == '.')) return (uint64_t)0;
-        uint32_t j = i;
-        while (j < n && b[j] == '.') ++j;
-        return (uint64_t)((j - i) / 3);
-      });
+      int64_t sum_chars = 0, alpha = 0, stop = 0;
+      uint64_t he = 0;
+      if constexpr (!kGqExt) {
+        const DevStopSet& ss = plan.stops[ds.stop_set];
+        const UcdView ucd = x.ucd;
+        gq_word_stats(x.par, W, [&](uint32_t k, uint32_t f) {
+          const uint32_t a = w.cs[k], e = w.ce[k];
+          return gq_word_term(ucd, ss, c, a, e, e - a, w.bs[k], w.be[k], (uint32_t)w.alpha[k], f);
+        }, sum_chars, alpha, stop);
+        x.stamp(PH_GQ_WORDS);
+        he = P::kWaves <= 1 ? gq_byte_counts(x.par, b, n) : gq_byte_counts_plain(x.par, b, n);
+      }
       x.stamp(PH_GQ_BYTES);
       const int64_t nhash = hi32(he), nell = lo32(he);
       const uint64_t be = x.par.template sum<uint64_t>(L.n, [&](uint32_t k) {
@@ -2690,15 +2776,15 @@
       });
       const int64_t bullet = hi32(be), ell_lines = lo32(be);
       x.par.single([&]() {
-        r[0] = W; r[1] = sum_chars; r[2] = nhash; r[3] = nell; r[4] = L.n;
-        r[5] = bullet; r[6] = ell_lines; r[7] = alpha; r[8] = stop;
+        if constexpr (!kGqExt) { r[0] = W; r[1] = sum_chars; r[2] = nhash; r[3] = nell; r[7] = alpha; r[8] = stop; }
+        r[4] = L.n; r[5] = bullet; r[6] = ell_lines;
       });
       x.stamp(PH_GQ);
-    } else if (ds.kind == DK_GOPHER_REP) {
+    } else if (kGr && ds.kind == DK_GOPHER_REP) {
       ++gr_seen;
       gopher_rep_record(x, ds, b, c, ph, w, r, kHotProps && gr_seen == n_gr, n_gr == 1 ? out.gr_export : nullptr,
-                        kPre ? out.pre : nullptr, out.b_global, L);
-    } else if (ds.kind == DK_FINEWEB) {
+                        kPre ? out.pre : nullptr, out.b_global, L, kGqExt);
+    } else if (kFw && ds.kind == DK_FINEWEB) {
       const auto mark = x.mark();
       uint32_t* nb = x.template alloc<uint32_t>(L.n + 1);
       if (x.overflow) { x.set_flag(DOC_NEEDS_CPU | DOC_OVERFLOW); return; }
diff --git a/csrc/hip/kernels.hip b/csrc/hip/kernels.hip
--- a/csrc/hip/kernels.hip
+++ b/csrc/hip/kernels.hip
@@ -70,7 +70,7 @@
   if (x.par.leader() && src[0] >= 0) src[0] += slice_begin;
 }
 
-#define TB_STAGE_KERNEL(NAME, ATTR)                                                                   \
+#define TB_STAGE_KERNEL(NAME, ATTR, KINDS)                                                                  \
   __global__ __launch_bounds__(64) ATTR void NAME(                                                   \
       const DevPlan* __restrict__ plan, const DevStage* __restrict__ stage, const uint8_t* __restrict__ bytes, \
       const int64_t* __restrict__ off, const int32_t* __restrict__ perm, int32_t ndocs, char* scratch,        \
@@ -87,13 +87,36 @@
     if (line_stats) out.line_stats = line_stats + line_stats_base(off[doc], doc);                     \
     if (gr_export) { out.gr_export = gr_export + blockIdx.x; out.b_global = bytes + off[doc]; }       \
     out.dict = dict;                                                                                  \
-    analyze_stage<WavePar, false>(x, *stage, *plan, LidTables{}, b, n, out);  \
+    analyze_stage<WavePar, false, false, KINDS>(x, *stage, *plan, LidTables{}, b, n, out);  \
   }
 
 #ifndef TB_STAGE_WPE
 #define TB_STAGE_WPE 8
 #endif
-TB_STAGE_KERNEL(k_stage_analyze_wave, __attribute__((amdgpu_waves_per_eu(TB_STAGE_WPE, 8))))
+#define TB_STAGE_ATTR __attribute__((amdgpu_waves_per_eu(TB_STAGE_WPE, 8)))
+TB_STAGE_KERNEL(k_stage_analyze_wave, TB_STAGE_ATTR, SK_ALL)
+TB_STAGE_KERNEL(k_stage_wave_gr_gqx, TB_STAGE_ATTR, SK_GR | SK_GQ | SK_GQ_EXT)
+TB_STAGE_KERNEL(k_stage_wave_gr, TB_STAGE_ATTR, SK_GR)
+TB_STAGE_KERNEL(k_stage_wave_fw, TB_STAGE_ATTR, SK_FW)
+
+#ifndef TB_GQ_SWAR
+#define TB_GQ_SWAR 0
+#endif
+__global__ __launch_bounds__(64) void k_gq_wave(
+    const DevPlan* __restrict__ plan, const DevStage* __restrict__ stage, int32_t gq_step,
+    const uint8_t* __restrict__ bytes, const int64_t* __restrict__ off, const int32_t* __restrict__ perm,
+    int32_t ndocs, const GrExport* __restrict__ ex, DevTables tabs, int64_t* rec) {
+  const int doc = perm[blockIdx.x];
+  if (doc >= ndocs) return;
+  const GrExport& e = ex[blockIdx.x];
+  if (!e.gq_valid) return;
+  WavePar par;
+  const DevStep& ds = stage->steps[gq_step];
+  int64_t* r = rec + (int64_t)ds.rec_prefix * ndocs + (int64_t)doc * ds.width;
+  const uint32_t n = (uint32_t)(off[doc + 1] - off[doc]);
+  gq_export_record<TB_GQ_SWAR != 0>(par, UcdView{tabs.s1, tabs.s2, tabs.l1, tabs.l2}, plan->stops[ds.stop_set], e,
+                                    bytes + off[doc], n, r);
+}
 
 #ifndef TB_BLOCK_THREADS
 #define TB_BLOCK_THREADS 512
@@ -1493,6 +1516,14 @@
 
 int tb_scan_strided_i64(hipStream_t stream, const int64_t* src, int64_t stride, int64_t n, int64_t* out);
 
+int tb_stage_analyze_variant(hipStream_t stream, const void* plan, const void* stage, const uint8_t* bytes,
+                             const int64_t* off, const int32_t* perm, int32_t ndocs, char* scratch,
+                             const int64_t* scratch_off, const uint64_t* pw, uint32_t pw_n, const uint16_t* s1,
+                             const uint32_t* s2, const uint16_t* l1, const int32_t* l2, int64_t* rec, uint32_t* flags,
+                             uint32_t lds_bytes, uint64_t* prof, int32_t waves, int32_t nblocks, const uint8_t* dead,
+                             uint32_t* line_stats, void* gr_export, const int64_t* dict_moff,
+                             const uint32_t* dict_bits, const uint32_t* dict_words, int32_t variant);
+
 int tb_stage_analyze(hipStream_t stream, const void* plan, const void* stage, const uint8_t* bytes,
                      const int64_t* off, const int32_t* perm, int32_t ndocs, char* scratch,
                      const int64_t* scratch_off, const uint64_t* pw, uint32_t pw_n, const uint16_t* s1,
@@ -1500,17 +1531,45 @@
                      uint32_t lds_bytes, uint64_t* prof, int32_t waves, int32_t nblocks, const uint8_t* dead,
                      uint32_t* line_stats, void* gr_export, const int64_t* dict_moff, const uint32_t* dict_bits,
                      const uint32_t* dict_words) {
+  return tb_stage_analyze_variant(stream, plan, stage, bytes, off, perm, ndocs, scratch, scratch_off, pw, pw_n, s1, s2,
+                                  l1, l2, rec, flags, lds_bytes, prof, waves, nblocks, dead, line_stats, gr_export,
+                                  dict_moff, dict_bits, dict_words, SV_GENERIC);
+}
+
+int tb_stage_analyze_variant(hipStream_t stream, const void* plan, const void* stage, const uint8_t* bytes,
+                             const int64_t* off, const int32_t* perm, int32_t ndocs, char* scratch,
+                             const int64_t* scratch_off, const uint64_t* pw, uint32_t pw_n, const uint16_t* s1,
+                             const uint32_t* s2, const uint16_t* l1, const int32_t* l2, int64_t* rec, uint32_t* flags,
+                             uint32_t lds_bytes, uint64_t* prof, int32_t waves, int32_t nblocks, const uint8_t* dead,
+                             uint32_t* line_stats, void* gr_export, const int64_t* dict_moff,
+                             const uint32_t* dict_bits, const uint32_t* dict_words, int32_t variant) {
   if (ndocs <= 0) return 0;
   if (nblocks <= 0) nblocks = ndocs;
   if (lds_bytes > kMaxLdsPerDoc) return (int)hipErrorInvalidValue;
   DevTables t{s1, s2, l1, l2};
   if (waves != TB_STAGE_WPE) return (int)hipErrorInvalidValue;
-  auto kern = k_stage_analyze_wave;
+  if (variant < 0 || variant >= SV_COUNT || (variant == SV_GR_GQX && !gr_export)) return (int)hipErrorInvalidValue;
+  auto kern = variant == SV_GR_GQX ? k_stage_wave_gr_gqx
+              : variant == SV_GR   ? k_stage_wave_gr
+              : variant == SV_FW   ? k_stage_wave_fw
+                                   : k_stage_analyze_wave;
   if (lds_bytes > 65536)
     (void)hipFuncSetAttribute((const void*)kern, hipFuncAttributeMaxDynamicSharedMemorySize, (int)lds_bytes);
   hipLaunchKernelGGL(kern, dim3(nblocks), dim3(64), lds_bytes, stream, (const DevPlan*)plan,
                      (const DevStage*)stage, bytes, off, perm, ndocs, scratch, scratch_off, pw, pw_n, t, rec, flags,
                      lds_bytes, prof, dead, line_stats, (GrExport*)gr_export, DictIn{dict_moff, dict_bits, dict_words});
+  return (int)hipGetLastError();
+}
+
+int tb_gq_wave(hipStream_t stream, const void* plan, const void* stage, int32_t gq_step, const uint8_t* bytes,
+               const int64_t* off, const int32_t* perm, int32_t n_docs, int32_t ndocs, const void* gr_export,
+               const uint16_t* s1, const uint32_t* s2, const uint16_t* l1, const int32_t* l2, int64_t* rec) {
+  if (n_docs <= 0) return 0;
+  if (!plan || !stage || !bytes || !off || !perm || !gr_export || !rec || gq_step < 0 || gq_step >= kMaxStageSteps)
+    return (int)hipErrorInvalidValue;
+  hipLaunchKernelGGL(k_gq_wave, dim3((uint32_t)n_docs), dim3(64), 0, stream, (const DevPlan*)plan,
+                     (const DevStage*)stage, gq_step, bytes, off, perm, ndocs, (const GrExport*)gr_export,
+                     DevTables{s1, s2, l1, l2}, rec);
   return (int)hipGetLastError();
 }
 
@@ -1773,7 +1832,7 @@
 int tb_phase_slots() { return kPhaseSlots; }
 int tb_stage_waves() { return TB_STAGE_WPE; }
 
-int tb_abi_version() { return 24; }
+int tb_abi_version() { return 25; }
 size_t tb_sizeof_plan() { return sizeof(DevPlan); }
 size_t tb_sizeof_stage() { return sizeof(DevStage); }
 size_t tb_sizeof_c4() { return sizeof(DevC4); }
diff --git a/csrc/host/devplan_build.cpp b/csrc/host/devplan_build.cpp
--- a/csrc/host/devplan_build.cpp
+++ b/csrc/host/devplan_build.cpp
@@ -339,6 +339,10 @@
   int gr_pos = -1;
   for (int s = 0; s < st.n_steps; ++s)
     if (st.steps[s].kind == DK_GOPHER_REP) gr_pos = s;
+  const int32_t variant = stage_variant(st);
+  int gq_pos = -1;
+  for (int s = 0; s < st.n_steps; ++s)
+    if (st.steps[s].kind == DK_GOPHER_QUALITY) gq_pos = s;
   bool has_lid = false;
   for (int s = 0; s < st.n_steps; ++s) has_lid |= st.steps[s].kind == DK_LANGID;
   if (has_lid && !lid) { delete plan; throw std::runtime_error("language model required"); }
@@ -372,7 +376,18 @@
       if (line_stats) out.line_stats = line_stats + line_stats_base(off[i], i);
       GrExport ex{};
       if (split_tasks > 0 && gr_pos >= 0) out.gr_export = &ex;
-      analyze_stage(x, st, *plan, lid ? lid->tables() : LidTables{}, (const uint8_t*)data + off[i], n, out);
+      const LidTables lt = lid ? lid->tables() : LidTables{};
+      const uint8_t* text = (const uint8_t*)data + off[i];
+      if (out.gr_export && variant == SV_GR_GQX) {
+        analyze_stage<SeqPar, true, false, SK_GR | SK_GQ | SK_GQ_EXT | SK_LID>(x, st, *plan, lt, text, n, out);
+        if (ex.gq_valid) {
+          const DevStep& gq = st.steps[gq_pos];
+          gq_export_record<true>(x.par, ucd, plan->stops[gq.stop_set], ex, text, n,
+                                 rec.data() + (int64_t)gq.rec_prefix * ndocs + i * gq.width);
+        }
+      } else {
+        analyze_stage(x, st, *plan, lt, text, n, out);
+      }
       if (x.overflow) continue;
       if (!out.gr_export || !ex.valid) {
         note_scratch(x.peak, n);
diff --git a/csrc/host/module.cpp b/csrc/host/module.cpp
--- a/csrc/host/module.cpp
+++ b/csrc/host/module.cpp
@@ -836,6 +836,17 @@
     for (int i = 0; i < d.n_steps; ++i) out.append(py::make_tuple(d.steps[i].kind, d.steps[i].width, d.steps[i].rec_prefix));
     return py::make_tuple(d.width_total, out);
   });
+  m.def("stage_variant", [](const py::bytes& b) {
+    std::string s = b;
+    if (s.size() < sizeof(DevStage)) throw std::runtime_error("stage_variant: not a DevStage blob");
+    DevStage d;
+    std::memcpy(&d, s.data(), sizeof(d));
+    return (int)stage_variant(d);
+  });
+  m.attr("SV_GENERIC") = (int)SV_GENERIC;
+  m.attr("SV_GR_GQX") = (int)SV_GR_GQX;
+  m.attr("SV_GR") = (int)SV_GR;
+  m.attr("SV_FW") = (int)SV_FW;
   m.def("pow_table", [](uint32_t n) { return to_numpy(pow_table(n)); });
   m.def("scratch_bytes_for", [](uint32_t n, bool split) { return scratch_bytes_for(n, split); }, py::arg("n"),
         py::arg("split") = false);
diff --git a/textblaster_amd/ops/kernels.py b/textblaster_amd/ops/kernels.py
--- a/textblaster_amd/ops/kernels.py
+++ b/textblaster_amd/ops/kernels.py
@@ -13,11 +13,14 @@
 _I64 = ctypes.c_int64
 _SZ = ctypes.c_size_t
 
-ABI_VERSION = 24
+ABI_VERSION = 25
 
 _SIGS = {
     "tb_stage_analyze": [_P, _P, _P, _P, _P, _P, _I32, _P, _P, _P, _U32, _P, _P, _P, _P, _P, _P, _U32, _P, _I32, _I32, _P,
                          _P, _P, _P, _P, _P],
+    "tb_stage_analyze_variant": [_P, _P, _P, _P, _P, _P, _I32, _P, _P, _P, _U32, _P, _P, _P, _P, _P, _P, _U32, _P, _I32,
+                                 _I32, _P, _P, _P, _P, _P, _P, _I32],
+    "tb_gq_wave": [_P, _P, _P, _I32, _P, _P, _P, _I32, _I32, _P, _P, _P, _P, _P, _P],
     "tb_gr_split_wave": [_P, _P, _I32, _P, _I32, _I32, _I32, _P, _P, _U32, _P, _P, _P, _P, _P, _P, _U32, _I32, _P,
                          _I32],
     "tb_c4_pass_a": [_P, _P, _P, _P, _P, _I32, _P, _P, _P, _U32, _P, _P, _P, _P, _P, _P, _P, _U32, _P, _I32, _P, _P,
@@ -164,16 +167,25 @@
 
     def stage_analyze(self, plan, stage, bytes_, off, perm, ndocs, scratch, scratch_off, pw, pw_n, rec, flags,
                       lds_bytes=0, prof=None, waves=0, nblocks=0, dead=None, line_stats=None, gr_export=None,
-                      dict_in=None):
+                      dict_in=None, variant=0):
         t = self.tabs
         if gr_export is not None and gr_export.nbytes < max(nblocks, 0) * self.sizeof_gr_export:
             raise DeviceError("stage_analyze: export buffer too small")
-        rc = self.lib.tb_stage_analyze(
+        rc = self.lib.tb_stage_analyze_variant(
             self.stream(), plan.data_ptr(), stage.data_ptr(), bytes_.data_ptr(), off.data_ptr(), _ptr(perm), ndocs,
             scratch.data_ptr(), scratch_off.data_ptr(), pw.data_ptr(), pw_n, t[0].data_ptr(), t[1].data_ptr(),
             t[2].data_ptr(), t[3].data_ptr(), rec.data_ptr(), flags.data_ptr(), lds_bytes, _ptr(prof), waves, nblocks,
-            _ptr(dead), _ptr(line_stats), _ptr(gr_export), *_dict_ptrs(dict_in))
+            _ptr(dead), _ptr(line_stats), _ptr(gr_export), *_dict_ptrs(dict_in), int(variant))
         _check(rc, "tb_stage_analyze")
+
+    def gq_wave(self, plan, stage, gq_step, bytes_, off, perm, n_docs, ndocs, gr_export, rec):
+        if gr_export.nbytes < n_docs * self.sizeof_gr_export or perm.numel() < n_docs:
+            raise DeviceError("gq_wave: operand shapes")
+        t = self.tabs
+        rc = self.lib.tb_gq_wave(self.stream(), plan.data_ptr(), stage.data_ptr(), int(gq_step), bytes_.data_ptr(),
+                                 off.data_ptr(), perm.data_ptr(), n_docs, ndocs, gr_export.data_ptr(),
+                                 t[0].data_ptr(), t[1].data_ptr(), t[2].data_ptr(), t[3].data_ptr(), rec.data_ptr())
+        _check(rc, "tb_gq_wave")
 
     def gr_export_wave_bytes(self, n_docs: int) -> int:
         return n_docs * self.sizeof_gr_export + 16 + 4 * n_docs
diff --git a/textblaster_amd/pipeline/device.py b/textblaster_amd/pipeline/device.py
--- a/textblaster_amd/pipeline/device.py
+++ b/textblaster_amd/pipeline/device.py
@@ -378,6 +378,7 @@
             self.plan_t = self._to_dev(plan_b)
             self.stage_ts = [self._to_dev(b) for b in stage_bs]
             self.stage_layout = [h.stage_layout(b) for b in stage_bs]
+            self.stage_variant = [int(h.stage_variant(b)) for b in stage_bs]
             self.c4_ts = {i: self._to_dev(h.build_c4(steps_native[i])) for i in plan.c4_steps}
             self.has_lid = any(steps_native[i].kind == h.StepKind.LanguageDetection
                                for st in plan.stages for i in st)
@@ -811,7 +812,11 @@
                         self.k.stage_analyze(self.plan_t, self.stage_ts[s], vb, vo, d_perm[n_long:], ndocs,
                                              scratch, d_soff[n_long:], pw, pw_n, rec, flags,
                                              self.lds_bytes, prof, self.stage_waves, nw, skip, ls_out, gxw,
-                                             dict_in.get(ver))
+                                             dict_in.get(ver), self.stage_variant[s])
+                        if self.stage_variant[s] == h.SV_GR_GQX:
+                            gq_pos = [k for k, (kind, _, _) in enumerate(layout) if kind == KIND_GOPHER_QUALITY][0]
+                            self.k.gq_wave(self.plan_t, self.stage_ts[s], gq_pos, vb, vo, d_perm[n_long:], nw, ndocs,
+                                           gxw, rec)
                         if gxw is not None:
                             gr_pos, n_tasks = self.gr_split[s]
                             n_big = int(np.count_nonzero(lens_perm[n_long:] > self.ngram_big_bytes))
```

Result: slower. 12.83 million (-2.8%).
